# linkedin/ml-ease

Hardware: NVIDIA H100
Metric: ADMM iterations/sec (higher is better)
Workload: dtype f32 data / f64 reductions / bf16 (dense) or e4m3 (CSR) Gram operands

## Files before the change

### ml-ease_b200/csrc/batch.cu

```cuda
#include <algorithm>
#include <cstring>
#include <string>
#include <vector>

#include "host.cuh"

namespace mlease {

namespace {

__global__ void poll2_kernel(const Problem* probs, int nprob, int* flag_out, Problem* compact) {
  __shared__ int s_cnt;
  if (threadIdx.x == 0) s_cnt = 0;
  __syncthreads();
  int running = 0, emit = 0;
  for (int b = threadIdx.x; b < nprob; b += blockDim.x) {
    const Ctrl* c = probs[b].ctrl;
    if (!c->done) {
      running = 1;
      if (c->emit) { emit = 1; compact[atomicAdd(&s_cnt, 1)] = probs[b]; }
    }
  }
  running = __syncthreads_or(running);
  emit = __syncthreads_or(emit);
  if (threadIdx.x == 0) { flag_out[0] = running | (emit << 1); flag_out[1] = s_cnt; }
}

}

static int csr_operand_bytes(int csr_gram) { return csr_gram == CSR_GRAM_SPARSE ? 4 : 1; }
static double gram_path_bytes(const Batch& B) {
  const double Dp = round_up(B.ldx, 128), ldh = round_up(B.Dt, 32);
  double per = Dp * Dp * 4.0 + 3.0 * ldh * ldh * 8.0 + 2.0 * ldh * 32 * 8.0 + (cholesky_factored_direction((int)ldh) ? ldh * ldh * 2.0 : 0.0);
  double bytes = per * B.nprob;
  for (auto& p : B.h) bytes += (double)csr_operand_bytes(B.csr_gram) * (double)p.bm_entries;
  return bytes;
}

constexpr double GRAM_WGMMA_S_PER_MAC = 1.317e-15, GRAM_WGMMA_S_PER_READ = 4.315e-12;
constexpr double GRAM_SPARSE_S_PER_PAIR = 1.808e-12, GRAM_SPARSE_S_PER_VISIT = 2.548e-10, GRAM_SPARSE_S_PER_READ = 2.915e-12;
static double gram_cost(const Problem& p, int Dp, int kind, double ctas, int num_sms) {
  const double nblk = Dp / 128, tiles = nblk * (nblk + 1) / 2, groups = (double)((p.n + 31) / 32);
  const int span = gram_sparse_span(p.bm_entries, Dp / 128, (p.n + 31) / 32);
  const double spans = (double)(((p.n + 31) / 32 + span - 1) / span);
  const double reads = (nblk + 1) * (double)p.bm_entries;
  if (kind == CSR_GRAM_WGMMA) return tiles * 128.0 * 128.0 * 32.0 * groups * GRAM_WGMMA_S_PER_MAC + reads * GRAM_WGMMA_S_PER_READ;
  return (p.gram_pairs * GRAM_SPARSE_S_PER_PAIR + tiles * spans * GRAM_SPARSE_S_PER_VISIT + reads * GRAM_SPARSE_S_PER_READ) *
         std::max(1.0, num_sms / std::max(1.0, ctas));
}

int batch_alloc(Batch& B, int num_sms, int hessian_policy, int csr_gram_force) {
  const int nprob = B.nprob, ldx = B.ldx;
  B.Dp = round_up(B.ldx, 128);
  B.ldh = round_up(B.Dt, 32);
  long long maxn = 1;
  for (auto& p : B.h) maxn = std::max(maxn, p.n);
  int R = 64, cps = 1;
  if (!B.csr) {
    int S, G;
    size_t smem;
    if (!k1_dense_plan(ldx, &R, &S, &G, &smem, &cps))
      return fail(MLEASE_ERR_INVALID, "dense partitions support at most 4095 features (+intercept); use CSR input beyond that");
  }
  const long long row_tiles = (maxn + R - 1) / R;
  B.k1_dyn = (nprob > 1 && nprob <= 32) ? nprob : 0;
  if (B.k1_dyn) B.k1_grid = (int)std::max(1LL, std::min((long long)num_sms * cps, (long long)nprob * row_tiles));
  else B.k1_grid = (int)std::max(1LL, std::min(row_tiles, (long long)std::max(1, (num_sms * cps) / std::max(1, nprob))));
  B.gram_from_csr = B.csr ? 1 : 0;
  for (auto& p : B.h) if (!p.bm_offs) B.gram_from_csr = 0;
  B.csr_fx = B.gram_from_csr;
  if (hessian_policy == 2 && B.csr) {
    B.csr_fx = 1;
    for (auto& p : B.h) if (!p.csr_unique) B.csr_fx = 0;
  }
  B.k1_fused = 0;
  if (B.csr && B.csr_fx && B.group_L >= 1 && B.group_L <= 4 && nprob % B.group_L == 0) {
    bool ok = true;
    for (auto& p : B.h) if (!p.sg_perm || p.sg_S != B.h[0].sg_S || p.sg_rows != B.h[0].sg_rows) ok = false;
    if (ok) {
      B.k1f_LP = B.group_L <= 1 ? 1 : (B.group_L == 2 ? 2 : 4);
      B.k1f_smem = (size_t)ldx * 4 * B.k1f_LP + (size_t)B.h[0].sg_rows * 4 * B.k1f_LP;
      if (B.k1f_smem <= 224 * 1024) { B.k1_fused = 1; B.k1_dyn = 0; B.k1_grid = B.h[0].sg_S; }
    }
  }
  const int gpart_rows = B.k1_fused ? 1 : B.k1_grid;
  if (hessian_policy == 2 && !B.csr)
    return fail(MLEASE_ERR_INVALID, "hessian_policy 2 (matrix-free Newton-CG) needs CSR partitions; dense partitions (at most 4095 features) use the Gram path");
  if (hessian_policy == 2 && !B.csr_fx)
    return fail(MLEASE_ERR_INVALID, "hessian_policy 2 (matrix-free Newton-CG) needs CSR rows with strictly increasing column ids");
  B.matfree = hessian_policy == 2 ? 1 : 0;
  B.csr_gram = 0;
  if (B.gram_from_csr && !B.matfree) {
    double t_sparse = 0, t_wgmma = 0;
    bool fits = true;
    const double nblk = B.Dp / 128, ctas = nblk * (nblk + 1) / 2 * nprob;
    for (auto& p : B.h) {
      t_sparse += gram_cost(p, B.Dp, CSR_GRAM_SPARSE, ctas, num_sms);
      t_wgmma += gram_cost(p, B.Dp, CSR_GRAM_WGMMA, ctas, num_sms);
      if (p.n > gram_sparse_max_rows()) fits = false;
    }
    B.csr_gram = (fits && t_sparse < t_wgmma) ? CSR_GRAM_SPARSE : CSR_GRAM_WGMMA;
    if (csr_gram_force == CSR_GRAM_SPARSE && !fits)
      return fail(MLEASE_ERR_INVALID, "the sparse CSR Gram's int64 sums hold at most 2^27 rows per partition");
    if (csr_gram_force) B.csr_gram = csr_gram_force;
  }
  if (!B.matfree && B.csr && B.gram_from_csr) {
    double state = 0;
    for (auto& p : B.h) state += 8.0 * (double)p.n;
    state += (double)nprob * (8.0 * ((9 + 2 * BFGS_M + gpart_rows) * (double)ldx + B.k1_grid + 8) + 16.0 * ldx +
                              (B.k1_fused ? 4.0 * B.k1_grid * ldx : 0.0));
    size_t free_b = 0, total_b = 0;
    CK(cudaMemGetInfo(&free_b, &total_b));
    if (gram_path_bytes(B) + state + (256.0 * 1024 * 1024) > (double)free_b) { B.matfree = 1; B.csr_gram = 0; }
  }
  {
    double bytes = 0;
    for (auto& p : B.h) bytes = std::max(bytes, B.csr ? 8.0 * (double)p.nnz_hint + 17.0 * (double)p.n : (double)p.n * 4.0 * ldx);
    const double t_pass = bytes / 5e12 + 20e-6;
    const double t_rebuild = (double)maxn * B.Dt * B.Dt / 1e15 + (double)B.Dt * B.Dt * B.Dt / 5e12 + 300e-6;
    B.rebuild_is_expensive = (t_rebuild > 8.0 * t_pass && B.Dt > 2048 && !B.matfree) ? 1 : 0;
  }
  constexpr int MAX_TILES = 1 << 18;
  std::vector<short> tiles(B.matfree ? 2 : 2 * (size_t)MAX_TILES);
  B.ntiles = B.matfree ? 0 : gram_tile_list(B.Dp, tiles.data(), MAX_TILES, B.csr_gram == CSR_GRAM_SPARSE ? 2 : B.gram_from_csr);
  if (B.ntiles <= 0 && !B.matfree) return fail(MLEASE_ERR_INVALID, "Gram tile list overflow");
  if (!B.matfree && B.csr_gram != CSR_GRAM_SPARSE) {
    const long long ksteps = (maxn + 63) / 64;
    const long long base = (long long)B.ntiles * nprob;
    const long long cap = std::max(1, num_sms);
    int best = 1;
    double best_eff = 0;
    for (int s = 1; s <= 16; s++) {
      if (s > ksteps) break;
      const long long ctas = base * s;
      const double eff = (double)ctas / (double)(((ctas + cap - 1) / cap) * cap);
      if (eff > best_eff + 1e-9) { best_eff = eff; best = s; }
      if (eff >= 0.93 && ctas >= 2LL * cap) { best = s; break; }
    }
    while (best > 1 && (double)best * B.Dp * B.Dp * 4.0 * nprob > 1024.0 * 1024 * 1024) best--;
    B.gram_slices = best;
  }
  const size_t nd_prob = ((9 + (B.matfree ? 5 : 2 * BFGS_M)) * (size_t)ldx + 2 * BFGS_M + (size_t)gpart_rows * ldx + (size_t)B.k1_grid + 8 + 3) & ~(size_t)3;
  const size_t nd = (size_t)nprob * nd_prob;
  const size_t nf = (size_t)nprob * 4 * ldx;
  double* dd; float* ff; float* hp = nullptr; double* lc = nullptr; double* ld = nullptr; double* ldi = nullptr; double* yi = nullptr; double* hi = nullptr;
  if (int rc = B.mem.get(&dd, nd, true)) return rc;
  if (int rc = B.mem.get(&ff, nf, true)) return rc;
  float* gpf = nullptr;
  if (B.k1_fused)
    if (int rc = B.mem.get(&gpf, (size_t)nprob * B.k1_grid * ldx, true)) return rc;
  __nv_bfloat16* hif = nullptr;
  if (!B.matfree) {
    if (int rc = B.mem.get(&hp, (size_t)nprob * B.gram_slices * B.Dp * B.Dp, true)) return rc;
    if (int rc = B.mem.get(&lc, (size_t)nprob * B.ldh * B.ldh, true)) return rc;
    if (int rc = B.mem.get(&ld, (size_t)nprob * B.ldh * 32, true)) return rc;
    if (int rc = B.mem.get(&ldi, (size_t)nprob * B.ldh * 32, true)) return rc;
    if (int rc = B.mem.get(&yi, (size_t)nprob * B.ldh * B.ldh, true)) return rc;
    if (int rc = B.mem.get(&hi, (size_t)nprob * B.ldh * B.ldh, true)) return rc;
    if (cholesky_factored_direction(B.ldh))
      if (int rc = B.mem.get(&hif, (size_t)nprob * B.ldh * B.ldh, true)) return rc;
  }
  if (int rc = B.mem.get(&B.d_ctrl, (size_t)nprob, true)) return rc;
  if (int rc = B.mem.get(&B.d, (size_t)nprob, true)) return rc;
  if (nprob > 64 || B.lockstep)
    if (int rc = B.mem.get(&B.d_compact, (size_t)nprob, true)) return rc;
  if (int rc = B.mem.get(&B.d_tmaps, nprob, true)) return rc;
  if (int rc = B.mem.get(&B.d_tiles, (size_t)B.ntiles * 2, true)) return rc;
  CK(cudaMemcpy(B.d_tiles, tiles.data(), (size_t)B.ntiles * 2 * sizeof(short), cudaMemcpyHostToDevice));
  std::vector<CUtensorMap> maps(nprob);
  std::vector<size_t> pool_off(nprob);
  size_t pool_bytes = 0;
  for (int b = 0; b < nprob; b++) {
    pool_off[b] = pool_bytes;
    const bool windows = B.csr_fx && k1_csr_window(ldx) > 0;
    const size_t need = B.csr_fx ? (((size_t)B.h[b].n * sizeof(float) * (windows ? 2 : 1) + 255) & ~(size_t)255) +
                                       (B.matfree ? 0 : (size_t)csr_operand_bytes(B.csr_gram) * (size_t)B.h[b].bm_entries)
                                        : (size_t)B.h[b].n * B.Dp * sizeof(__nv_bfloat16);
    pool_bytes += (need + 255) & ~(size_t)255;
  }
  unsigned char* pool = nullptr;
  if (int rc = B.mem.get(&pool, pool_bytes, true)) return rc;
  for (int b = 0; b < nprob; b++) {
    Problem& p = B.h[b];
    p.ldx = ldx; p.Dt = B.Dt; p.Dp = B.Dp; p.ldh = B.ldh; p.self_idx = b;
    p.k1_ctas = B.k1_grid;
    p.gram_slices = B.gram_slices;
    double* const q0 = dd;
    double* q = dd;
    p.beta = q; q += ldx; p.beta_t = q; q += ldx; p.m = q; q += ldx; p.q = q; q += ldx;
    p.g_t = q; q += ldx; p.g_acc = q; q += ldx; p.dir = q; q += ldx; p.x_d = q; q += ldx;
    p.qf = reinterpret_cast<float*>(q); p.tf = p.qf + ldx; q += ldx;
    if (!B.matfree) { p.bfgs_S = q; q += (size_t)BFGS_M * ldx; p.bfgs_Y = q; q += (size_t)BFGS_M * ldx; }
    p.bfgs_rho = q; q += BFGS_M; p.bfgs_alpha = q; q += BFGS_M;
    p.gpart = q; q += (size_t)gpart_rows * ldx;
    p.hv_vf = p.qf;
    if (B.matfree) { p.cg_r = q; q += ldx; p.cg_p = q; q += ldx; p.cg_z = q; q += ldx; p.cg_Hp = q; q += ldx; p.cg_diag = q; q += ldx; }
    p.gpart_f = gpf ? gpf + (size_t)b * B.k1_grid * ldx : nullptr;
    p.fpart = q; q += B.k1_grid + 8;
    dd = q0 + nd_prob;
    float* f = ff;
    p.beta_tf = f; f += ldx; p.u_f = f; f += ldx; p.uplusx_f = f; f += ldx; p.x_f = f; f += ldx;
    ff = f;
    p.Hpart = hp ? hp + (size_t)b * B.gram_slices * B.Dp * B.Dp : nullptr;
    p.Lc = lc ? lc + (size_t)b * B.ldh * B.ldh : nullptr;
    p.Ldiag = ld ? ld + (size_t)b * B.ldh * 32 : nullptr;
    p.Ldinv = ldi ? ldi + (size_t)b * B.ldh * 32 : nullptr;
    p.Yinv = yi ? yi + (size_t)b * B.ldh * B.ldh : nullptr;
    p.Hinv = hi ? hi + (size_t)b * B.ldh * B.ldh : nullptr;
    p.Ysym = hif ? hif + (size_t)b * B.ldh * B.ldh : nullptr;
    p.ctrl = B.d_ctrl + b;
    if (B.csr_fx) {
      p.sdvec = reinterpret_cast<float*>(pool + pool_off[b]);
      p.rvec = k1_csr_window(ldx) > 0 ? p.sdvec + p.n : nullptr;
      unsigned char* op = B.matfree ? nullptr : pool + pool_off[b] + (((size_t)p.n * sizeof(float) * (p.rvec ? 2 : 1) + 255) & ~(size_t)255);
      p.bm_e4m3 = B.csr_gram == CSR_GRAM_SPARSE ? nullptr : op;
      p.bm_word = B.csr_gram == CSR_GRAM_SPARSE ? reinterpret_cast<uint32_t*>(op) : nullptr;
      p.gram_from_csr = B.gram_from_csr;
      p.csr_gram = B.csr_gram;
      std::memset(&maps[b], 0, sizeof(CUtensorMap));
    } else {
      p.gram_from_csr = 0;
      p.csr_gram = 0;
      p.gram_scale = 1.f; p.gram_unscale = 1.f;
      p.Xt = reinterpret_cast<__nv_bfloat16*>(pool + pool_off[b]);
      if (gram_make_tensor_map(&maps[b], p.Xt, p.n, B.Dp) != 0) return fail(MLEASE_ERR_CUDA, "cuTensorMapEncodeTiled failed");
    }
  }
  CK(cudaMemcpy(B.d_tmaps, maps.data(), (size_t)nprob * sizeof(CUtensorMap), cudaMemcpyHostToDevice));
  CK(cudaMemcpy(B.d, B.h.data(), (size_t)nprob * sizeof(Problem), cudaMemcpyHostToDevice));
  return 0;
}

cudaError_t batch_gram(const Batch& B, const Problem* d_probs, int n, int force, cudaStream_t st, int* launches, int share) {
  if (B.csr_gram == CSR_GRAM_SPARSE) return gram_launch_csr_sparse(d_probs, n, B.d_tiles, B.ntiles, force, st, launches, share);
  if (B.gram_from_csr) return gram_launch_csr_wgmma(d_probs, n, B.d_tiles, B.ntiles, B.gram_slices, force, st, launches, share);
  return gram_launch_wgmma(d_probs, n, B.d_tmaps, B.d_tiles, B.ntiles, B.gram_slices, force, st, launches, share);
}

static double gram_build_flops(const Batch& B, const Problem& p) {
  return B.csr_gram == CSR_GRAM_SPARSE ? 2.0 * p.gram_pairs : (double)p.n * (double)B.Dt * (double)(B.Dt + 1);
}

cudaError_t batch_k1(Batch& B, int force_emit, cudaStream_t st, int* launches, int mode) {
  if (mode != K1_GRAD && !(B.csr && B.csr_fx)) return cudaErrorInvalidValue;
  if (B.k1_fused)
    return k1f_launch(B.d, B.nprob / B.group_L, B.group_L, B.h[0].sg_S, B.k1f_LP, B.k1f_smem, B.has_bias, force_emit, st, launches, mode);
  return k1_launch(B.d, B.nprob, B.csr, B.ldx, B.has_bias, B.k1_grid, force_emit, st, launches, B.csr_fx, B.k1_dyn, mode);
}

int batch_factor(Batch& B, const Problem* d_hess, int n_hess, int share, bool share_fact, int skip_prep, cudaStream_t st, int* launches) {
  if (B.ysym_shared) CK(cholesky_detach_followers(B.d, B.nprob, B.ldh, st, launches));
  if (share_fact) CK(cholesky_share_begin(B.d, B.nprob, share, st, launches));
  CK(cholesky_launch(d_hess, n_hess, B.ldh, st, launches, share, skip_prep));
  if (share_fact) {
    CK(cholesky_share_end(B.d, B.nprob, share, st, launches));
    if (cholesky_factored_direction(B.ldh)) B.ysym_shared = true;
    const size_t hh = (size_t)B.ldh * B.ldh;
    for (int b = 0; b < B.nprob; b++) {
      if (b % share == 0) continue;
      const Problem& lead = B.h[b - b % share];
      if (!cholesky_factored_direction(B.ldh)) CK(cudaMemcpyAsync(B.h[b].Hinv, lead.Hinv, hh * sizeof(double), cudaMemcpyDeviceToDevice, st));
    }
  }
  B.has_factor = true;
  return 0;
}

static int mf_direction(Batch& B, const SlotCtx& x) {
  constexpr int CG_CHUNK = 4;
  Profiler& pf = *x.pf;
  cudaStream_t st = x.st;
  int& launches = *x.launches;
  pf.begin(2, st);
  CK(cg_begin(B.d, B.nprob, st, &launches));
  CK(batch_k1(B, 0, st, &launches, K1_DIAG));
  CK(hv_reduce(B.d, B.nprob, B.Dt, 2, st, &launches));
  CK(cg_init(B.d, B.nprob, B.Dt, st, &launches));
  pf.end(st);
  for (int steps = 0; steps < CG_MAX_STEPS; steps += CG_CHUNK) {
    for (int j = 0; j < CG_CHUNK; j++) {
      pf.begin(2, st);
      CK(batch_k1(B, 0, st, &launches, K1_HV));
      CK(hv_reduce(B.d, B.nprob, B.Dt, 1, st, &launches));
      CK(cg_step(B.d, B.nprob, B.Dt, st, &launches));
      pf.end(st);
    }
    CK(cg_poll(B.d, B.nprob, x.d_flag + 2, st, &launches));
    CK(cudaMemcpyAsync(x.h_flag + 2, x.d_flag + 2, sizeof(int), cudaMemcpyDeviceToHost, st));
    CK(cudaStreamSynchronize(st));
    if (!x.h_flag[2]) break;
  }
  return 0;
}

int batch_slot(Batch& B, const SlotCtx& x, int slot_idx, bool with_hess, bool spec) {
  Profiler& pf = *x.pf;
  cudaStream_t st = x.st;
  int& launches = *x.launches;
  pf.begin(0, st);
  CK(batch_k1(B, B.matfree ? 1 : -1, st, &launches));
  pf.end(st);
  pf.begin(1, st);
  CK(k1_reduce_decide(B.d, B.nprob, B.Dt, st, &launches, spec ? 1 : 0));
  pf.end(st);
  if (with_hess && x.n_hess > 0) {
    pf.begin(2, st);
    const int share = (slot_idx == 0) ? x.share_first_gram : 0;
    if (share > 1)
      for (int b = 0; b < B.nprob; b++) if (b % share != 0) *x.shared_flops += gram_build_flops(B, B.h[b]);
    CK(batch_gram(B, x.d_hess, x.n_hess, 0, st, &launches, share));
    pf.end(st);
    pf.begin(3, st);
    const bool share_fact = share > 1 && x.share_first_factor;
    if (int rc = batch_factor(B, x.d_hess, x.n_hess, share, share_fact, 0, st, &launches)) return rc;
    pf.end(st);
  }
  if (B.matfree)
    if (int rc = mf_direction(B, x)) return rc;
  pf.begin(1, st);
  if (B.matfree) CK(newton_finish(B.d, B.nprob, B.Dt, st, &launches));
  else CK(newton_solve(B.d, B.nprob, B.ldh, st, &launches, B.group_L));
  if (x.poll) { poll2_kernel<<<1, 256, 0, st>>>(B.d, B.nprob, x.d_flag, B.d_compact); launches++; }
  pf.end(st);
  return 0;
}

int batch_xupdate(Batch& B, cudaStream_t st, double xtol, int max_newton, int policy, int invalidate, int* h_flag, int* d_flag,
                  Counters& cnt, Profiler* prof, int share_first_gram, int share_first_factor) {
  Profiler nop;
  Profiler& pf = prof ? *prof : nop;
  int launches = 0;
  if (B.matfree) policy = 2;
  CK(newton_begin(B.d, B.nprob, xtol, max_newton, policy, invalidate, B.rebuild_is_expensive, st, &launches));
  const bool small = B.nprob <= 64 && !B.lockstep;
  int flag = 1;
  {
    bool emit0 = policy == 1 || invalidate || B.mirror.empty();
    for (auto& c : B.mirror) if (!c.hess_valid || c.refresh_next) emit0 = true;
    if (emit0 && !B.matfree) flag |= 2;
  }
  B.mirror.resize(B.nprob);
  std::vector<Ctrl>& hc = B.mirror;
  int slots = 0;
  const Problem* d_hess = B.d;
  int n_hess = B.nprob;
  double shared_flops = 0;
  auto enqueue_slot = [&](int slot_idx, bool with_hess, bool spec) -> int {
    const SlotCtx x{st, &pf, &launches, d_hess, n_hess, share_first_gram, share_first_factor, &shared_flops, h_flag, d_flag, !small};
    return batch_slot(B, x, slot_idx, with_hess, spec);
  };
  if (small) {
    for (int i = 0; i < 2; i++) {
      if (!B.h_ctrl[i]) if (int rc = B.pinned.get(&B.h_ctrl[i], B.nprob, false)) return rc;
      if (!B.slot_ev[i]) CK(cudaEventCreateWithFlags(&B.slot_ev[i], cudaEventDisableTiming));
    }
    const bool may_spec = policy == 0;
    auto flags_of = [&](const Ctrl* c, bool* all_valid) {
      int f = 0; bool v = true;
      for (int b = 0; b < B.nprob; b++) if (!c[b].done) { f |= 1; if (c[b].emit) f |= 2; if (!c[b].hess_valid) v = false; }
      *all_valid = v;
      return f;
    };
    auto finish_slot = [&](int idx) -> int {
      CK(cudaMemcpyAsync(B.h_ctrl[idx & 1], B.d_ctrl, (size_t)B.nprob * sizeof(Ctrl), cudaMemcpyDeviceToHost, st));
      CK(cudaEventRecord(B.slot_ev[idx & 1], st));
      return 0;
    };
    bool known_valid = !(flag & 2);
    if (int rc = enqueue_slot(0, (flag & 2) != 0, false)) return rc;
    if (int rc = finish_slot(0)) return rc;
    int s_cur = 0;
    bool next_in_flight = false;
    int known_flag = flag;
    while (true) {
      const bool spec_next = may_spec && known_valid && !(known_flag & 2) && s_cur + 1 < 400;
      if (spec_next) {
        if (int rc = enqueue_slot(s_cur + 1, false, true)) return rc;
        if (int rc = finish_slot(s_cur + 1)) return rc;
        next_in_flight = true;
      }
      CK(cudaEventSynchronize(B.slot_ev[s_cur & 1]));
      std::memcpy(hc.data(), B.h_ctrl[s_cur & 1], (size_t)B.nprob * sizeof(Ctrl));
      slots = s_cur + 1;
      known_flag = flags_of(hc.data(), &known_valid);
      if (!(known_flag & 1) || slots >= 400) break;
      if (next_in_flight) { s_cur++; next_in_flight = false; continue; }
      if (int rc = enqueue_slot(s_cur + 1, (known_flag & 2) != 0, false)) return rc;
      if (int rc = finish_slot(s_cur + 1)) return rc;
      s_cur++;
    }
    flag = known_flag;
  }
  while (!small && (flag & 1) && slots < 400) {
    if (int rc = enqueue_slot(slots, (flag & 2) != 0, false)) return rc;
    CK(cudaMemcpyAsync(h_flag, d_flag, 2 * sizeof(int), cudaMemcpyDeviceToHost, st));
    CK(cudaStreamSynchronize(st));
    flag = h_flag[0];
    n_hess = h_flag[1];
    d_hess = B.d_compact;
    slots++;
  }
  if (!small) {
    CK(cudaMemcpyAsync(hc.data(), B.d_ctrl, (size_t)B.nprob * sizeof(Ctrl), cudaMemcpyDeviceToHost, st));
    CK(cudaStreamSynchronize(st));
  }
  cnt.launches += launches;
  cnt.last_slots = slots;
  int bad_spd = 0, bad_ls = 0;
  if (pf.on) CK(cudaStreamSynchronize(st));
  pf.resolve();
  for (int b = 0; b < B.nprob; b++) {
    const Ctrl& c = hc[b];
    const Problem& p = B.h[b];
    const double rowbytes = B.csr ? 17.0 : (4.0 * B.ldx + 9.0);
    cnt.k1_bytes += (double)c.evals * ((double)p.n * rowbytes + (B.csr ? 8.0 * (double)p.nnz_hint : 0.0));
    cnt.gram_flops += (double)c.hess_builds * gram_build_flops(B, p);
    cnt.k1_emit_bytes += (double)c.hess_builds * (double)p.n * (double)B.Dp * 2.0;
  }
  cnt.gram_flops -= shared_flops;
  if (B.csr) {
    const int gl = std::max(1, B.group_L);
    for (int g0 = 0; g0 + gl <= B.nprob; g0 += gl) {
      int mx = 0; long long sum = 0;
      for (int l = 0; l < gl; l++) { mx = std::max(mx, hc[g0 + l].evals); sum += hc[g0 + l].evals; }
      const Problem& p = B.h[g0];
      cnt.k1_shared_bytes += (double)mx * (8.0 * (double)p.nnz_hint + 9.0 * (double)p.n) + (double)sum * 8.0 * (double)p.n;
    }
  }
  for (auto& c : hc) {
    cnt.k1_passes += c.evals; cnt.newton_steps += c.newton_steps; cnt.rejected += c.rejects; cnt.gram_builds += c.hess_builds;
    if (c.fail == 3 || !c.done) cnt.not_converged++;
    if (c.fail == 1) bad_spd++;
    if (c.fail == 2) bad_ls++;
  }
  if (bad_spd) return fail(MLEASE_ERR_NUMERIC, "Model fitting error! (Hessian not positive definite in " + std::to_string(bad_spd) + " problem(s))");
  if (bad_ls) return fail(MLEASE_ERR_NUMERIC, "Model fitting error! (line search failed in " + std::to_string(bad_ls) + " problem(s))");
  return 0;
}

}
```

### ml-ease_b200/csrc/common.cuh

```cuda
#pragma once
#include <cuda_bf16.h>
#include <cuda_runtime.h>
#include <stdint.h>

namespace mlease {

constexpr int BFGS_M = 6;
constexpr int CG_MAX_STEPS = 64;

struct Ctrl {
  int done;
  int have_dir;
  int need_solve;
  int need_hess;
  int emit;
  int hess_valid;
  int fail;
  int newton_steps;
  int evals;
  int rejects;
  int hess_builds;
  int stall;
  int bfgs_count;
  double h0_scale;
  int k1_chunks;
  int refresh_next;
  int skip_eval;
  int warm_used;
  int build_step;
  double worst_ratio;
  double alpha;
  double phi0;
  double f_acc, f_t;
  double gnorm;
  double gnorm_prev;
  double dirnorm;
  double dirnorm_prev;
  double xtol;
  int max_newton;
  int hess_policy;
  int rebuild_is_expensive;
  long long tot_evals, tot_newton, tot_rejects, tot_hess;
  const void* ysym_use;
  int cg_active;
  int cg_iter;
  double cg_rz;
  double cg_g2;
  float hv_vinf;
};

enum { K1_GRAD = 0, K1_HV = 1, K1_DIAG = 2 };
enum { CSR_GRAM_WGMMA = 1, CSR_GRAM_SPARSE = 2 };

struct Problem {
  const float* X;
  long long n;
  int ldx;
  int Dt;
  const signed char* y;
  const float* w;
  const float* o;
  const long long* rowptr;
  const int* colidx;
  const float* vals;
  long long nnz_hint;
  int csr_unique;
  const long long* bm_offs;
  const unsigned short* bm_keys;
  const float* bm_vals;
  long long bm_groups;
  long long bm_entries;
  unsigned char* bm_e4m3;
  uint32_t* bm_word;
  float vmax, wmax;
  int nblk128;
  int sg_S, sg_rows, sg_ngrp;
  const int* sg_perm;
  const int* sg_depth;
  const long long* sg_goff;
  const unsigned short* sg_row16;
  const float* sg_val;
  const unsigned short* sg_col16;
  float* gpart_f;
  float* sdvec;
  float* rvec;
  int gram_from_csr;
  int csr_gram;
  double gram_pairs;
  float gram_scale;
  float gram_unscale;
  __nv_bfloat16* Xt;
  int Dp;
  double* beta;
  double* beta_t;
  float* beta_tf;
  double* m;
  double* q;
  double* g_t;
  double* g_acc;
  double* dir;
  double* gpart;
  double* fpart;
  int k1_ctas;
  float* Hpart;
  int gram_slices;
  double* Lc;
  double* Ldiag;
  double* Ldinv;
  double* Yinv;
  double* Hinv;
  __nv_bfloat16* Ysym;
  float* qf;
  float* tf;
  int ldh;
  Ctrl* ctrl;
  float* u_f;
  float* uplusx_f;
  float* x_f;
  double* bfgs_S;
  double* bfgs_Y;
  double* bfgs_rho;
  double* bfgs_alpha;
  double* x_d;
  int lambda_idx;
  int self_idx;
  int part_local;
  float rowl1;
  float* hv_vf;
  double* cg_r;
  double* cg_p;
  double* cg_z;
  double* cg_Hp;
  double* cg_diag;
};

__device__ __forceinline__ uint32_t smem_u32(const void* p) { return (uint32_t)__cvta_generic_to_shared(p); }

__device__ __forceinline__ void mbar_init(uint64_t* bar, uint32_t count) {
  asm volatile("mbarrier.init.shared::cta.b64 [%0], %1;" ::"r"(smem_u32(bar)), "r"(count) : "memory");
}
__device__ __forceinline__ void fence_mbar_init() { asm volatile("fence.mbarrier_init.release.cluster;" ::: "memory"); }
__device__ __forceinline__ void fence_proxy_async_smem() { asm volatile("fence.proxy.async.shared::cta;" ::: "memory"); }
__device__ __forceinline__ void mbar_arrive_expect_tx(uint64_t* bar, uint32_t bytes) {
  asm volatile("mbarrier.arrive.expect_tx.shared::cta.b64 _, [%0], %1;" ::"r"(smem_u32(bar)), "r"(bytes) : "memory");
}
__device__ __forceinline__ void mbar_arrive(uint64_t* bar) {
  asm volatile("mbarrier.arrive.shared::cta.b64 _, [%0];" ::"r"(smem_u32(bar)) : "memory");
}
__device__ __forceinline__ bool mbar_try_wait(uint64_t* bar, uint32_t parity) {
  uint32_t ok;
  asm volatile(
      "{\n"
      ".reg .pred p;\n"
      "mbarrier.try_wait.parity.shared::cta.b64 p, [%1], %2;\n"
      "selp.u32 %0, 1, 0, p;\n"
      "}\n"
      : "=r"(ok)
      : "r"(smem_u32(bar)), "r"(parity)
      : "memory");
  return ok != 0;
}
__device__ __forceinline__ void mbar_wait(uint64_t* bar, uint32_t parity) {
  while (!mbar_try_wait(bar, parity)) {
  }
}
__device__ __forceinline__ void mbar_arrive(uint32_t bar) { asm volatile("mbarrier.arrive.shared::cta.b64 _, [%0];" ::"r"(bar) : "memory"); }
__device__ __forceinline__ void mbar_wait(uint32_t bar, uint32_t parity) {
  uint32_t ok;
  do {
    asm volatile(
        "{\n"
        ".reg .pred p;\n"
        "mbarrier.try_wait.parity.shared::cta.b64 p, [%1], %2;\n"
        "selp.u32 %0, 1, 0, p;\n"
        "}\n"
        : "=r"(ok)
        : "r"(bar), "r"(parity)
        : "memory");
  } while (!ok);
}

__device__ __forceinline__ void sts_u8(uint32_t saddr, uint32_t v) { asm volatile("st.shared.u8 [%0], %1;" ::"r"(saddr), "r"(v) : "memory"); }
__device__ __forceinline__ void bulk_g2s(void* dst_smem, const void* src_gmem, uint32_t bytes, uint64_t* bar) {
  asm volatile("cp.async.bulk.shared::cluster.global.mbarrier::complete_tx::bytes [%0], [%1], %2, [%3];" ::"r"(
                   smem_u32(dst_smem)),
               "l"(src_gmem), "r"(bytes), "r"(smem_u32(bar))
               : "memory");
}

__device__ __forceinline__ void tma_load_2d(void* dst_smem, const void* tmap, int c0, int c1, uint64_t* bar) {
  asm volatile(
      "cp.async.bulk.tensor.2d.shared::cluster.global.tile.mbarrier::complete_tx::bytes [%0], [%1, {%2, %3}], [%4];" ::"r"(
          smem_u32(dst_smem)),
      "l"(tmap), "r"(c0), "r"(c1), "r"(smem_u32(bar))
      : "memory");
}
__device__ __forceinline__ void tma_prefetch_desc(const void* tmap) {
  asm volatile("prefetch.tensormap [%0];" ::"l"(tmap) : "memory");
}

__device__ __forceinline__ uint64_t wgmma_desc(uint32_t smem_addr, uint32_t lbo_bytes, uint32_t sbo_bytes, uint32_t layout) {
  uint64_t d = 0;
  d |= (uint64_t)((smem_addr & 0x3FFFF) >> 4);
  d |= (uint64_t)((lbo_bytes >> 4) & 0x3FFF) << 16;
  d |= (uint64_t)((sbo_bytes >> 4) & 0x3FFF) << 32;
  d |= (uint64_t)(layout & 3) << 62;
  return d;
}
__device__ __forceinline__ void wgmma_fence() { asm volatile("wgmma.fence.sync.aligned;" ::: "memory"); }
__device__ __forceinline__ void wgmma_commit() { asm volatile("wgmma.commit_group.sync.aligned;" ::: "memory"); }
template <int N>
__device__ __forceinline__ void wgmma_wait() { asm volatile("wgmma.wait_group.sync.aligned %0;" ::"n"(N) : "memory"); }
__device__ __forceinline__ void wgmma_bf16_m64n256k16_tt(float (&d)[128], uint64_t desc_a, uint64_t desc_b) {
  asm volatile(
      "{\n"
      ".reg .pred p;\n"
      "setp.ne.b32 p, 1, 0;\n"
      "wgmma.mma_async.sync.aligned.m64n256k16.f32.bf16.bf16 {"
      "%0, %1, %2, %3, %4, %5, %6, %7, %8, %9, %10, %11, %12, %13, %14, %15, "
      "%16, %17, %18, %19, %20, %21, %22, %23, %24, %25, %26, %27, %28, %29, %30, %31, "
      "%32, %33, %34, %35, %36, %37, %38, %39, %40, %41, %42, %43, %44, %45, %46, %47, "
      "%48, %49, %50, %51, %52, %53, %54, %55, %56, %57, %58, %59, %60, %61, %62, %63, "
      "%64, %65, %66, %67, %68, %69, %70, %71, %72, %73, %74, %75, %76, %77, %78, %79, "
      "%80, %81, %82, %83, %84, %85, %86, %87, %88, %89, %90, %91, %92, %93, %94, %95, "
      "%96, %97, %98, %99, %100, %101, %102, %103, %104, %105, %106, %107, %108, %109, %110, %111, "
      "%112, %113, %114, %115, %116, %117, %118, %119, %120, %121, %122, %123, %124, %125, %126, %127}, "
      "%128, %129, p, 1, 1, 1, 1;\n"
      "}\n"
      : "+f"(d[0]), "+f"(d[1]), "+f"(d[2]), "+f"(d[3]), "+f"(d[4]), "+f"(d[5]), "+f"(d[6]), "+f"(d[7]),
        "+f"(d[8]), "+f"(d[9]), "+f"(d[10]), "+f"(d[11]), "+f"(d[12]), "+f"(d[13]), "+f"(d[14]), "+f"(d[15]),
        "+f"(d[16]), "+f"(d[17]), "+f"(d[18]), "+f"(d[19]), "+f"(d[20]), "+f"(d[21]), "+f"(d[22]), "+f"(d[23]),
        "+f"(d[24]), "+f"(d[25]), "+f"(d[26]), "+f"(d[27]), "+f"(d[28]), "+f"(d[29]), "+f"(d[30]), "+f"(d[31]),
        "+f"(d[32]), "+f"(d[33]), "+f"(d[34]), "+f"(d[35]), "+f"(d[36]), "+f"(d[37]), "+f"(d[38]), "+f"(d[39]),
        "+f"(d[40]), "+f"(d[41]), "+f"(d[42]), "+f"(d[43]), "+f"(d[44]), "+f"(d[45]), "+f"(d[46]), "+f"(d[47]),
        "+f"(d[48]), "+f"(d[49]), "+f"(d[50]), "+f"(d[51]), "+f"(d[52]), "+f"(d[53]), "+f"(d[54]), "+f"(d[55]),
        "+f"(d[56]), "+f"(d[57]), "+f"(d[58]), "+f"(d[59]), "+f"(d[60]), "+f"(d[61]), "+f"(d[62]), "+f"(d[63]),
        "+f"(d[64]), "+f"(d[65]), "+f"(d[66]), "+f"(d[67]), "+f"(d[68]), "+f"(d[69]), "+f"(d[70]), "+f"(d[71]),
        "+f"(d[72]), "+f"(d[73]), "+f"(d[74]), "+f"(d[75]), "+f"(d[76]), "+f"(d[77]), "+f"(d[78]), "+f"(d[79]),
        "+f"(d[80]), "+f"(d[81]), "+f"(d[82]), "+f"(d[83]), "+f"(d[84]), "+f"(d[85]), "+f"(d[86]), "+f"(d[87]),
        "+f"(d[88]), "+f"(d[89]), "+f"(d[90]), "+f"(d[91]), "+f"(d[92]), "+f"(d[93]), "+f"(d[94]), "+f"(d[95]),
        "+f"(d[96]), "+f"(d[97]), "+f"(d[98]), "+f"(d[99]), "+f"(d[100]), "+f"(d[101]), "+f"(d[102]), "+f"(d[103]),
        "+f"(d[104]), "+f"(d[105]), "+f"(d[106]), "+f"(d[107]), "+f"(d[108]), "+f"(d[109]), "+f"(d[110]), "+f"(d[111]),
        "+f"(d[112]), "+f"(d[113]), "+f"(d[114]), "+f"(d[115]), "+f"(d[116]), "+f"(d[117]), "+f"(d[118]), "+f"(d[119]),
        "+f"(d[120]), "+f"(d[121]), "+f"(d[122]), "+f"(d[123]), "+f"(d[124]), "+f"(d[125]), "+f"(d[126]), "+f"(d[127])
      : "l"(desc_a), "l"(desc_b)
      : "memory");
}
__device__ __forceinline__ void wgmma_e4m3_m64n128k32(float (&d)[64], uint64_t desc_a, uint64_t desc_b, uint32_t accumulate) {
  asm volatile(
      "{\n"
      ".reg .pred p;\n"
      "setp.ne.b32 p, %66, 0;\n"
      "wgmma.mma_async.sync.aligned.m64n128k32.f32.e4m3.e4m3 {"
      "%0, %1, %2, %3, %4, %5, %6, %7, %8, %9, %10, %11, %12, %13, %14, %15, "
      "%16, %17, %18, %19, %20, %21, %22, %23, %24, %25, %26, %27, %28, %29, %30, %31, "
      "%32, %33, %34, %35, %36, %37, %38, %39, %40, %41, %42, %43, %44, %45, %46, %47, "
      "%48, %49, %50, %51, %52, %53, %54, %55, %56, %57, %58, %59, %60, %61, %62, %63}, "
      "%64, %65, p, 1, 1;\n"
      "}\n"
      : "+f"(d[0]), "+f"(d[1]), "+f"(d[2]), "+f"(d[3]), "+f"(d[4]), "+f"(d[5]), "+f"(d[6]), "+f"(d[7]),
        "+f"(d[8]), "+f"(d[9]), "+f"(d[10]), "+f"(d[11]), "+f"(d[12]), "+f"(d[13]), "+f"(d[14]), "+f"(d[15]),
        "+f"(d[16]), "+f"(d[17]), "+f"(d[18]), "+f"(d[19]), "+f"(d[20]), "+f"(d[21]), "+f"(d[22]), "+f"(d[23]),
        "+f"(d[24]), "+f"(d[25]), "+f"(d[26]), "+f"(d[27]), "+f"(d[28]), "+f"(d[29]), "+f"(d[30]), "+f"(d[31]),
        "+f"(d[32]), "+f"(d[33]), "+f"(d[34]), "+f"(d[35]), "+f"(d[36]), "+f"(d[37]), "+f"(d[38]), "+f"(d[39]),
        "+f"(d[40]), "+f"(d[41]), "+f"(d[42]), "+f"(d[43]), "+f"(d[44]), "+f"(d[45]), "+f"(d[46]), "+f"(d[47]),
        "+f"(d[48]), "+f"(d[49]), "+f"(d[50]), "+f"(d[51]), "+f"(d[52]), "+f"(d[53]), "+f"(d[54]), "+f"(d[55]),
        "+f"(d[56]), "+f"(d[57]), "+f"(d[58]), "+f"(d[59]), "+f"(d[60]), "+f"(d[61]), "+f"(d[62]), "+f"(d[63])
      : "l"(desc_a), "l"(desc_b), "r"(accumulate)
      : "memory");
}

template <int N>
__device__ __forceinline__ void setmaxnreg_dec() { asm volatile("setmaxnreg.dec.sync.aligned.u32 %0;" ::"n"(N)); }
template <int N>
__device__ __forceinline__ void setmaxnreg_inc() { asm volatile("setmaxnreg.inc.sync.aligned.u32 %0;" ::"n"(N)); }

__device__ __forceinline__ float warp_sum(float v) {
#pragma unroll
  for (int o = 16; o > 0; o >>= 1) v += __shfl_xor_sync(0xffffffffu, v, o);
  return v;
}
__device__ __forceinline__ double warp_sum(double v) {
#pragma unroll
  for (int o = 16; o > 0; o >>= 1) v += __shfl_xor_sync(0xffffffffu, v, o);
  return v;
}
__device__ __forceinline__ double warp_max(double v) {
#pragma unroll
  for (int o = 16; o > 0; o >>= 1) v = fmax(v, __shfl_xor_sync(0xffffffffu, v, o));
  return v;
}

}
```

### ml-ease_b200/csrc/ingest.cu

```cuda
#include <algorithm>
#include <cstring>
#include <string>

#include "host.cuh"

namespace mlease {

namespace {

__global__ void fill_bias_pad_kernel(float* X, long long n, int ldx, int Dg, int has_bias) {
  const int npad = ldx - Dg;
  const long long total = n * npad;
  for (long long e = (long long)blockIdx.x * blockDim.x + threadIdx.x; e < total; e += (long long)gridDim.x * blockDim.x) {
    const long long i = e / npad;
    const int c = Dg + (int)(e % npad);
    X[i * ldx + c] = (c == Dg && has_bias) ? 1.0f : 0.0f;
  }
}
__global__ void convert_labels_kernel(long long n, const int* resp, const float* w_in, const float* o_in, signed char* y, float* w,
                                      float* o, int* bad) {
  for (long long i = (long long)blockIdx.x * blockDim.x + threadIdx.x; i < n; i += (long long)gridDim.x * blockDim.x) {
    const int r = resp[i];
    if (r != 1 && r != 0 && r != -1) atomicOr(bad, 1);
    y[i] = (r == 1) ? 1 : -1;
    const float ww = w_in ? w_in[i] : 1.0f;
    if (!(ww >= 0.f)) atomicOr(bad, 2);
    w[i] = ww;
    o[i] = o_in ? o_in[i] : 0.0f;
  }
}
__global__ void check_rows_sorted_kernel(long long n, const long long* rowptr, const int* colidx, int* bad) {
  for (long long i = (long long)blockIdx.x * blockDim.x + threadIdx.x; i < n; i += (long long)gridDim.x * blockDim.x)
    for (long long j = rowptr[i] + 1; j < rowptr[i + 1]; j++)
      if (colidx[j] <= colidx[j - 1]) { atomicOr(bad, 8); break; }
}
__global__ void absmax_kernel(long long n, const float* __restrict__ a, unsigned* __restrict__ out) {
  float m = 0.f;
  for (long long j = (long long)blockIdx.x * blockDim.x + threadIdx.x; j < n; j += (long long)gridDim.x * blockDim.x) m = fmaxf(m, fabsf(a[j]));
  m = warp_max(m);
  if ((threadIdx.x & 31) == 0) atomicMax(out, __float_as_uint(m));
}
__global__ void csr_gram_pairs_kernel(long long n, const long long* __restrict__ rowptr, unsigned long long* __restrict__ out) {
  unsigned long long s = 0;
  for (long long i = (long long)blockIdx.x * blockDim.x + threadIdx.x; i < n; i += (long long)gridDim.x * blockDim.x) {
    const unsigned long long k = (unsigned long long)(rowptr[i + 1] - rowptr[i]);
    s += (k + 1) * (k + 2) / 2;
  }
  for (int d = 16; d > 0; d >>= 1) s += __shfl_down_sync(0xffffffffu, s, d);
  if ((threadIdx.x & 31) == 0) atomicAdd(out, s);
}
__global__ void check_csr_kernel(long long nnz, const int* colidx, float* vals, int Dg, int binary, int* bad) {
  for (long long j = (long long)blockIdx.x * blockDim.x + threadIdx.x; j < nnz; j += (long long)gridDim.x * blockDim.x) {
    const int c = colidx[j];
    if (c < 0 || c >= Dg) atomicOr(bad, 4);
    if (binary) vals[j] = 1.0f;
  }
}
__global__ void gather_i64_kernel(const long long* src, const long long* idx, int n, long long* out) {
  const int i = blockIdx.x * blockDim.x + threadIdx.x;
  if (i < n) out[i] = src[idx[i]];
}
__global__ void rebase_rowptr_kernel(long long n, const long long* src, long long base, long long* dst) {
  for (long long i = (long long)blockIdx.x * blockDim.x + threadIdx.x; i <= n; i += (long long)gridDim.x * blockDim.x) dst[i] = src[i] - base;
}
__global__ void repack_rows_kernel(float* dst, int ldx, const float* src, long long ld_in, long long rows, int Dg) {
  const long long total = rows * Dg;
  for (long long e = (long long)blockIdx.x * blockDim.x + threadIdx.x; e < total; e += (long long)gridDim.x * blockDim.x) {
    const long long i = e / Dg;
    const int c = (int)(e - i * Dg);
    dst[i * ldx + c] = src[i * ld_in + c];
  }
}

}

bool is_device_ptr(const void* p) {
  cudaPointerAttributes a;
  const bool dev = cudaPointerGetAttributes(&a, p) == cudaSuccess && (a.type == cudaMemoryTypeDevice || a.type == cudaMemoryTypeManaged);
  cudaGetLastError();
  return dev;
}

bool is_dma_ptr(const void* p) {
  cudaPointerAttributes a;
  const bool dma = cudaPointerGetAttributes(&a, p) == cudaSuccess &&
                   (a.type == cudaMemoryTypeDevice || a.type == cudaMemoryTypeManaged || a.type == cudaMemoryTypeHost);
  cudaGetLastError();
  return dma;
}

int gather_rowptr(const int64_t* rowptr, const std::vector<long long>& idx, std::vector<long long>& out) {
  out.resize(idx.size());
  if (!is_device_ptr(rowptr)) {
    for (size_t i = 0; i < idx.size(); i++) out[i] = rowptr[idx[i]];
    return 0;
  }
  DevMem t;
  long long *d_idx, *d_out;
  if (int rc = t.get(&d_idx, idx.size(), false)) return rc;
  if (int rc = t.get(&d_out, idx.size(), false)) return rc;
  CK(cudaMemcpy(d_idx, idx.data(), idx.size() * 8, cudaMemcpyHostToDevice));
  gather_i64_kernel<<<(int)((idx.size() + 255) / 256), 256>>>((const long long*)rowptr, d_idx, (int)idx.size(), d_out);
  CK(cudaMemcpy(out.data(), d_out, idx.size() * 8, cudaMemcpyDeviceToHost));
  return 0;
}

int ingest_labels(cudaStream_t st, long long n, const int32_t* response, const float* weight, const float* offset, signed char* y, float* w,
                  float* o, int* d_flag, int* h_flag, float* wmax) {
  DevMem t;
  const int* d_r; const float *d_w, *d_o;
  if (int rc = to_device(t, (const int*)response, (size_t)n, &d_r, st)) return rc;
  if (int rc = to_device(t, weight, (size_t)n, &d_w, st)) return rc;
  if (int rc = to_device(t, offset, (size_t)n, &d_o, st)) return rc;
  CK(cudaMemsetAsync(d_flag, 0, 8, st));
  if (n > 0) {
    convert_labels_kernel<<<(int)std::min<long long>((n + 255) / 256, 4096), 256, 0, st>>>(n, d_r, d_w, d_o, y, w, o, d_flag);
    if (wmax) absmax_kernel<<<(int)std::min<long long>((n + 255) / 256, 2048), 256, 0, st>>>(n, w, (unsigned*)(d_flag + 1));
  }
  CK(cudaMemcpyAsync(h_flag, d_flag, 8, cudaMemcpyDeviceToHost, st));
  CK(cudaStreamSynchronize(st));
  if (h_flag[0] & 1) return fail(MLEASE_ERR_INVALID, "response (only 1, 0, -1 are allowed)");
  if (h_flag[0] & 2) return fail(MLEASE_ERR_INVALID, "weight cannot < 0");
  if (wmax && n > 0) std::memcpy(wmax, h_flag + 1, 4);
  return 0;
}

void check_csr(cudaStream_t st, long long n, long long nnz, const long long* rowptr, const int* colidx, float* vals, int Dg, int binary,
               int* d_flag) {
  if (nnz <= 0) return;
  check_csr_kernel<<<(int)std::min<long long>((nnz + 255) / 256, 4096), 256, 0, st>>>(nnz, colidx, vals, Dg, binary, d_flag);
  check_rows_sorted_kernel<<<(int)std::min<long long>((n + 255) / 256, 4096), 256, 0, st>>>(n, rowptr, colidx, d_flag + 1);
}

void rebase_rowptr(cudaStream_t st, long long n, const long long* src, long long base, long long* dst) {
  rebase_rowptr_kernel<<<(int)std::min<long long>((n + 256) / 256, 4096), 256, 0, st>>>(n, src, base, dst);
}

int upload_dense_rows(float* dst, int ldx, const float* src, long long ld_in, long long n, int Dg, int has_bias, cudaStream_t st) {
  if (is_device_ptr(src)) {
    repack_rows_kernel<<<4096, 256, 0, st>>>(dst, ldx, src, ld_in, n, Dg);
  } else {
    const long long chunk_rows = std::max<long long>(1, (128LL << 20) / (ld_in * 4));
    struct Staging {
      cudaEvent_t h2d_done[2] = {nullptr, nullptr}, repack_done[2] = {nullptr, nullptr};
      cudaStream_t cs = nullptr;
      ~Staging() {
        for (int b = 0; b < 2; b++) { if (h2d_done[b]) cudaEventDestroy(h2d_done[b]); if (repack_done[b]) cudaEventDestroy(repack_done[b]); }
        if (cs) cudaStreamDestroy(cs);
      }
    } sg;
    DevMem bufs;
    float* buf[2];
    CK(cudaStreamCreateWithFlags(&sg.cs, cudaStreamNonBlocking));
    for (int b = 0; b < 2; b++) {
      if (int rc = bufs.get(&buf[b], (size_t)chunk_rows * ld_in, false)) return rc;
      CK(cudaEventCreateWithFlags(&sg.h2d_done[b], cudaEventDisableTiming));
      CK(cudaEventCreateWithFlags(&sg.repack_done[b], cudaEventDisableTiming));
    }
    int ci = 0;
    for (long long r0 = 0; r0 < n; r0 += chunk_rows, ci++) {
      const int b = ci & 1;
      const long long rows = std::min(chunk_rows, n - r0);
      if (ci >= 2) CK(cudaStreamWaitEvent(sg.cs, sg.repack_done[b], 0));
      const size_t bytes = ((size_t)(rows - 1) * ld_in + Dg) * 4;
      CK(cudaMemcpyAsync(buf[b], src + r0 * ld_in, bytes, cudaMemcpyHostToDevice, sg.cs));
      CK(cudaEventRecord(sg.h2d_done[b], sg.cs));
      CK(cudaStreamWaitEvent(st, sg.h2d_done[b], 0));
      repack_rows_kernel<<<2048, 256, 0, st>>>(dst + r0 * ldx, ldx, buf[b], ld_in, rows, Dg);
      CK(cudaEventRecord(sg.repack_done[b], st));
    }
    CK(cudaStreamSynchronize(sg.cs));
    CK(cudaStreamSynchronize(st));
  }
  fill_bias_pad_kernel<<<1024, 256, 0, st>>>(dst, n, ldx, Dg, has_bias);
  return 0;
}

int csr_build_layout(mlease_session* s, PartData& pd) {
  Problem& d = pd.data;
  if (d.nnz_hint <= 0) return 0;
  const long long nrows = d.n, nnz = d.nnz_hint;
  const std::string who = "partition " + std::to_string(pd.pid) + ": ";
  int* f = s->d_flag;
  CK(cudaMemsetAsync(f, 0, 24, s->stream));
  check_csr(s->stream, nrows, nnz, d.rowptr, d.colidx, const_cast<float*>(d.vals), s->Dg, s->cfg.binary_feature, f);
  absmax_kernel<<<(int)std::min<long long>((nnz + 255) / 256, 2048), 256, 0, s->stream>>>(nnz, d.vals, (unsigned*)(f + 2));
  CK(csr_row_l1_max(nrows, d.rowptr, d.vals, (unsigned*)(f + 3), s->stream));
  csr_gram_pairs_kernel<<<(int)std::min<long long>((nrows + 255) / 256, 2048), 256, 0, s->stream>>>(nrows, d.rowptr, (unsigned long long*)(f + 4));
  CK(cudaMemcpyAsync(s->h_flag, f, 24, cudaMemcpyDeviceToHost, s->stream));
  CK(cudaStreamSynchronize(s->stream));
  if (s->h_flag[0]) return fail(MLEASE_ERR_INVALID, who + "feature index out of range");
  d.csr_unique = s->h_flag[1] ? 0 : 1;
  std::memcpy(&d.vmax, s->h_flag + 2, 4);
  std::memcpy(&d.rowl1, s->h_flag + 3, 4);
  unsigned long long pairs = 0;
  std::memcpy(&pairs, s->h_flag + 4, 8);
  if (d.csr_unique && nnz + nrows < (1LL << 32) - 64 && s->cfg.hessian_policy != 2) {
    d.nblk128 = round_up(s->ldx, 128) / 128;
    d.bm_groups = (nrows + 31) / 32;
    d.bm_entries = nnz + nrows;
    long long* bo; unsigned short* bk; float* bv;
    if (int rc = s->mem.get(&bo, (size_t)d.nblk128 * d.bm_groups + 1, true)) return rc;
    if (int rc = s->mem.get(&bk, (size_t)d.bm_entries, true)) return rc;
    if (int rc = s->mem.get(&bv, (size_t)d.bm_entries, true)) return rc;
    CK(csr_bm_offsets(nrows, d.rowptr, d.colidx, s->Dg, d.nblk128, d.bm_groups, bo, s->stream));
    CK(csr_bm_fill(nrows, d.rowptr, d.colidx, d.vals, s->Dg, d.nblk128, d.bm_groups, bo, bk, bv, s->stream));
    d.bm_offs = bo; d.bm_keys = bk; d.bm_vals = bv;
    d.gram_pairs = (double)pairs;
  }
  if (d.csr_unique && nnz + nrows < (1LL << 32) - 64) {
    int S = 0, rows = 0, LP = 0; size_t smem = 0;
    if (k1f_plan(nrows, s->ldx, s->L, s->num_sms, &S, &rows, &LP, &smem)) {
      int *perm, *depth; long long* goff; unsigned short *row16, *col16; float* val; long long total;
      CK(k1f_build(nrows, s->Dg, nnz, d.rowptr, d.colidx, d.vals, S, rows, &d.sg_ngrp, &perm, &depth, &goff, &row16, &val, &total, &col16,
                   s->stream));
      d.sg_S = S; d.sg_rows = rows;
      d.sg_perm = perm; d.sg_depth = depth; d.sg_goff = goff; d.sg_row16 = row16; d.sg_val = val; d.sg_col16 = col16;
      for (void* p : {(void*)perm, (void*)depth, (void*)goff, (void*)row16, (void*)val, (void*)col16}) s->mem.adopt(p);
    }
  }
  return 0;
}

}
```

### ml-ease_b200/csrc/k2_gram.cu

```cuda
#include <cuda.h>
#include <cuda_fp8.h>

#include <algorithm>
#include <cub/device/device_scan.cuh>

#include "kernels.cuh"

namespace mlease {

constexpr int GM = 128;
constexpr int GN = 256;
constexpr int GK = 64;
constexpr int UK = 16;
constexpr int GSTAGES = 4;
constexpr int G_A_BYTES = GK * GM * 2;
constexpr int G_B_BYTES = GK * GN * 2;
constexpr int G_STAGE_BYTES = G_A_BYTES + G_B_BYTES;
constexpr int G_BOX_BYTES = GK * 64 * 2;
constexpr int G_THREADS = 384;
constexpr size_t G_SMEM = (size_t)GSTAGES * G_STAGE_BYTES + 1024  + 256 ;
constexpr uint32_t DESC_SW128 = 1, DESC_SW32 = 3;

struct GramTile { short bi, bj; };

template <int N>
__device__ __forceinline__ void store_acc(float* out, int Dp, int row0, int col0, const float (&d)[N / 2]) {
  const int lane = threadIdx.x & 31, w = (threadIdx.x >> 5) & 3;
  const int r = row0 + w * 16 + (lane >> 2);
  if (r + 8 >= Dp) return;
#pragma unroll
  for (int j = 0; j < N / 8; j++) {
    const int c = col0 + 8 * j + 2 * (lane & 3);
    if (c < Dp) {
      *reinterpret_cast<float2*>(out + (size_t)r * Dp + c) = make_float2(d[4 * j], d[4 * j + 1]);
      *reinterpret_cast<float2*>(out + (size_t)(r + 8) * Dp + c) = make_float2(d[4 * j + 2], d[4 * j + 3]);
    }
  }
}

__global__ void __launch_bounds__(G_THREADS, 1)
gram_wgmma_kernel(const Problem* __restrict__ probs, const CUtensorMap* __restrict__ tmaps, const GramTile* __restrict__ tiles,
                  int ntiles, int force, int share) {
  if (share > 1 && blockIdx.z % share != 0) return;
  const int pidx = blockIdx.z;
  const Problem& pb = probs[pidx];
  Ctrl* ctrl = pb.ctrl;
  if (!force && (ctrl->done || !ctrl->need_hess)) return;
  const CUtensorMap* tmap = &tmaps[pb.self_idx];
  const GramTile tile = tiles[blockIdx.x];
  const int slice = blockIdx.y, nslices = gridDim.y;
  const int Dp = pb.Dp;
  const long long ksteps_total = (pb.n + GK - 1) / GK;
  const long long per = (ksteps_total + nslices - 1) / nslices;
  const long long ks0 = slice * per;
  const long long ks1 = min(ksteps_total, ks0 + per);
  const int nk = (int)max(0LL, ks1 - ks0);

  extern __shared__ unsigned char g_smem_raw[];
  unsigned char* smem = reinterpret_cast<unsigned char*>((reinterpret_cast<uintptr_t>(g_smem_raw) + 1023) & ~uintptr_t(1023));
  uint64_t* full_bar = reinterpret_cast<uint64_t*>(smem + (size_t)GSTAGES * G_STAGE_BYTES);
  uint64_t* empty_bar = full_bar + GSTAGES;

  const int lane = threadIdx.x & 31, wg = threadIdx.x >> 7;

  if (threadIdx.x == 0) {
    tma_prefetch_desc(tmap);
    for (int s = 0; s < GSTAGES; s++) { mbar_init(&full_bar[s], 1); mbar_init(&empty_bar[s], 8); }
    fence_mbar_init();
  }
  __syncthreads();

  if (wg == 0) {
    if (threadIdx.x == 0) {
      for (int k = 0; k < nk; k++) {
        const int st = k % GSTAGES;
        if (k >= GSTAGES) mbar_wait(&empty_bar[st], (uint32_t)(((k / GSTAGES) - 1) & 1));
        unsigned char* a_dst = smem + (size_t)st * G_STAGE_BYTES;
        unsigned char* b_dst = a_dst + G_A_BYTES;
        mbar_arrive_expect_tx(&full_bar[st], G_STAGE_BYTES);
        const int krow = (int)((ks0 + k) * GK);
#pragma unroll
        for (int b = 0; b < GM / 64; b++) tma_load_2d(a_dst + b * G_BOX_BYTES, tmap, tile.bi * GM + b * 64, krow, &full_bar[st]);
#pragma unroll
        for (int b = 0; b < GN / 64; b++) tma_load_2d(b_dst + b * G_BOX_BYTES, tmap, tile.bj * GN + b * 64, krow, &full_bar[st]);
      }
    }
  } else {
    float acc[GN / 2];
#pragma unroll
    for (int j = 0; j < GN / 2; j++) acc[j] = 0.f;
    const uint32_t smem_base = smem_u32(smem);
    for (int k = 0; k < nk; k++) {
      const int st = k % GSTAGES;
      mbar_wait(&full_bar[st], (uint32_t)((k / GSTAGES) & 1));
      const uint32_t a_addr = smem_base + (uint32_t)(st * G_STAGE_BYTES + (wg - 1) * G_BOX_BYTES);
      const uint32_t b_addr = smem_base + (uint32_t)(st * G_STAGE_BYTES + G_A_BYTES);
      wgmma_fence();
#pragma unroll
      for (int kk = 0; kk < GK / UK; kk++)
        wgmma_bf16_m64n256k16_tt(acc, wgmma_desc(a_addr + kk * (UK * 128), G_BOX_BYTES, 1024, DESC_SW128),
                                 wgmma_desc(b_addr + kk * (UK * 128), G_BOX_BYTES, 1024, DESC_SW128));
      wgmma_commit();
      wgmma_wait<1>();
      if (k > 0 && lane == 0) mbar_arrive(&empty_bar[(k - 1) % GSTAGES]);
    }
    wgmma_wait<0>();
    store_acc<GN>(pb.Hpart + (size_t)slice * Dp * Dp, Dp, tile.bi * GM + (wg - 1) * 64, tile.bj * GN, acc);
  }
}

constexpr int SK = 32;
constexpr int SN = 128;
constexpr int S_BOX_BYTES = SK * 128;
constexpr int SPW = 2;
constexpr int NGRP = 4;
constexpr int SST = 2 * NGRP;
constexpr int S_STAGE_BYTES = SPW * S_BOX_BYTES;
constexpr int S_CONSUMER_WARPS = 8;
constexpr int S_THREADS = (S_CONSUMER_WARPS + SPW * NGRP) * 32;
constexpr int S_CHAIN = 4;
static_assert(SST == 2 * S_CHAIN, "the consumer loop runs two chains per pass over the ring");
constexpr int S_REG_PRODUCER = 72, S_REG_CONSUMER = 184;
constexpr size_t S_SMEM = (size_t)SST * S_STAGE_BYTES + 1024  + 512 ;

__device__ __forceinline__ uint32_t kmaj_off(int k, int col) {
  return (uint32_t)(col * 32 + ((((k >> 4) ^ (col >> 2)) & 1) << 4) + (k & 15));
}
__device__ __forceinline__ int kmaj_row(uint32_t key) { return (int)(((((key >> 4) ^ (key >> 7)) & 1) << 4) | (key & 15)); }

__global__ void __launch_bounds__(S_THREADS, 1)
gram_csr_wgmma_kernel(const Problem* __restrict__ probs, const GramTile* __restrict__ tiles, int ntiles, int force, int share) {
  if (share > 1 && blockIdx.z % share != 0) return;
  const Problem& pb = probs[blockIdx.z];
  Ctrl* ctrl = pb.ctrl;
  if (!force && (ctrl->done || !ctrl->need_hess)) return;
  const GramTile tile = tiles[blockIdx.x];
  const int slice = blockIdx.y, nslices = gridDim.y;
  const int Dp = pb.Dp;
  const long long ksteps_total = (pb.n + SK - 1) / SK;
  const long long per = (ksteps_total + nslices - 1) / nslices;
  const long long ks0 = slice * per;
  const long long ks1 = min(ksteps_total, ks0 + per);
  const int nk = (int)max(0LL, ks1 - ks0);

  extern __shared__ unsigned char g_smem_raw[];
  unsigned char* smem = reinterpret_cast<unsigned char*>((reinterpret_cast<uintptr_t>(g_smem_raw) + 1023) & ~uintptr_t(1023));
  uint64_t* full_bar = reinterpret_cast<uint64_t*>(smem + (size_t)SST * S_STAGE_BYTES);
  uint64_t* empty_bar = full_bar + SST;
  const uint32_t smem_base = smem_u32(smem);
  const uint32_t full_u32 = smem_base + (uint32_t)SST * S_STAGE_BYTES, empty_u32 = full_u32 + 8 * SST;
  const int warp = threadIdx.x >> 5, lane = threadIdx.x & 31;

  for (int e = threadIdx.x; e < SST * S_STAGE_BYTES / 16; e += S_THREADS) reinterpret_cast<uint4*>(smem)[e] = make_uint4(0u, 0u, 0u, 0u);
  if (threadIdx.x == 0) {
    for (int s = 0; s < SST; s++) { mbar_init(&full_bar[s], SPW); mbar_init(&empty_bar[s], S_CONSUMER_WARPS); }
    fence_mbar_init();
  }
  fence_proxy_async_smem();
  __syncthreads();

  if (warp < S_CONSUMER_WARPS) {
    setmaxnreg_inc<S_REG_CONSUMER>();
    const int wg = warp >> 2;
    float acc[SN / 2], chain[SN / 2];
#pragma unroll
    for (int j = 0; j < SN / 2; j++) acc[j] = 0.f;
    const uint64_t desc_a0 = wgmma_desc(smem_base + (uint32_t)(wg * 64 * SK), 16, 256, DESC_SW32);
    const uint64_t desc_b0 = wgmma_desc(smem_base + (uint32_t)S_BOX_BYTES, 16, 256, DESC_SW32);
    const uint32_t desc_hi = (uint32_t)(desc_a0 >> 32);
    uint32_t a_lo = (uint32_t)desc_a0, b_lo = (uint32_t)desc_b0;
    asm volatile("" : "+r"(a_lo), "+r"(b_lo));
    auto desc_a = [&](int st) { return ((uint64_t)desc_hi << 32) | (a_lo + (uint32_t)(st * S_STAGE_BYTES / 16)); };
    auto desc_b = [&](int st) { return ((uint64_t)desc_hi << 32) | (b_lo + (uint32_t)(st * S_STAGE_BYTES / 16)); };
    auto issue = [&](int st, uint32_t ph, uint64_t a, uint64_t b, uint32_t accumulate) {
      mbar_wait(full_u32 + 8 * st, ph);
      wgmma_fence();
      wgmma_e4m3_m64n128k32(chain, a, b, accumulate);
      wgmma_commit();
    };
    auto release = [&](int st) { if (lane == 0) mbar_arrive(empty_u32 + 8 * st); };
    auto promote = [&]() {
#pragma unroll
      for (int j = 0; j < SN / 2; j++) acc[j] += chain[j];
    };
    auto run_chain = [&](int s0, uint32_t ph) {
#pragma unroll
      for (int c = 0; c < S_CHAIN; c++) {
        issue(s0 + c, ph, desc_a(s0 + c), desc_b(s0 + c), c != 0 ? 1u : 0u);
        if (c > 0) { wgmma_wait<1>(); release(s0 + c - 1); }
      }
      wgmma_wait<0>();
      release(s0 + S_CHAIN - 1);
      promote();
    };
    const int nring = nk - nk % SST, nfull = nk - nk % S_CHAIN;
    uint32_t ph = 0;
    int k = 0;
    for (; k < nring; k += SST) {
      run_chain(0, ph);
      run_chain(S_CHAIN, ph);
      ph ^= 1u;
    }
    if (k < nfull) { run_chain(0, ph); k += S_CHAIN; }
    for (; k < nk; k++) {
      const int st = k % SST;
      issue(st, (uint32_t)(k / SST) & 1u, desc_a(st), desc_b(st), 0u);
      wgmma_wait<0>();
      release(st);
      promote();
    }
    store_acc<SN>(pb.Hpart + (size_t)slice * Dp * Dp, Dp, tile.bi * 128 + wg * 64, tile.bj * SN, acc);
  } else {
    setmaxnreg_dec<S_REG_PRODUCER>();
    const int pw = warp - S_CONSUMER_WARPS;
    const int grp = pw / SPW, strm = pw % SPW;
    const int blk = strm == 0 ? tile.bi : tile.bj;
    const bool valid = blk < pb.nblk128;
    const long long* __restrict__ my_offs = pb.bm_offs + (size_t)(valid ? blk : 0) * pb.bm_groups + ks0 + (lane & 1);
    const unsigned short* __restrict__ keys = pb.bm_keys;
    const unsigned char* __restrict__ bytes = pb.bm_e4m3;
    constexpr uint32_t NOKEY = 0xFFFFFFFFu;
    const bool fetch = valid && lane < 2;
    auto ld_offs = [&](int k) -> uint32_t { return (fetch && k < nk) ? (uint32_t)__ldg(my_offs + k) : 0u; };

    struct Run { uint32_t lo, hi, key[2], byte[2]; };
    struct Written { uint32_t lo, hi, key[2]; };
    auto take_offs = [&](Run& r, uint32_t o) { r.lo = __shfl_sync(0xffffffffu, o, 0); r.hi = __shfl_sync(0xffffffffu, o, 1); };
    auto ld_entries = [&](Run& r) {
#pragma unroll
      for (int q = 0; q < 2; q++) {
        const uint32_t e = r.lo + lane + 32 * q;
        r.key[q] = e < r.hi ? (uint32_t)__ldg(keys + e) : NOKEY;
        r.byte[q] = e < r.hi ? (uint32_t)__ldg(bytes + e) : 0u;
      }
    };
    Run r0, r1;
    Written w0 = {0u, 0u, {NOKEY, NOKEY}}, w1 = {0u, 0u, {NOKEY, NOKEY}};
    take_offs(r0, ld_offs(grp));
    take_offs(r1, ld_offs(grp + NGRP));
    uint32_t o_c = ld_offs(grp + 2 * NGRP);
    ld_entries(r0);
    ld_entries(r1);
    const uint32_t sbase0 = smem_base + (uint32_t)(grp * S_STAGE_BYTES + strm * S_BOX_BYTES), sbase1 = sbase0 + NGRP * S_STAGE_BYTES;
    const uint32_t full0 = full_u32 + 8 * grp, empty0 = empty_u32 + 8 * grp;
    auto use = [&](int k, uint32_t sbase, uint32_t full, uint32_t empty, bool refill, uint32_t ph, Run& r, Written& w) {
      if (refill) {
        mbar_wait(empty, ph);
#pragma unroll
        for (int q = 0; q < 2; q++)
          if (w.key[q] != NOKEY) sts_u8(sbase + w.key[q], 0u);
        for (uint32_t e0 = w.lo + 64; e0 < w.hi; e0 += 32) {
          const uint32_t e = e0 + lane;
          if (e < w.hi) sts_u8(sbase + (uint32_t)__ldg(keys + e), 0u);
        }
      }
#pragma unroll
      for (int q = 0; q < 2; q++)
        if (r.key[q] != NOKEY) sts_u8(sbase + r.key[q], r.byte[q]);
      for (uint32_t e0 = r.lo + 64; e0 < r.hi; e0 += 32) {
        const uint32_t e = e0 + lane;
        if (e < r.hi) sts_u8(sbase + (uint32_t)__ldg(keys + e), (uint32_t)__ldg(bytes + e));
      }
      fence_proxy_async_smem();
      __syncwarp();
      if (lane == 0) mbar_arrive(full);
      w.lo = r.lo; w.hi = r.hi; w.key[0] = r.key[0]; w.key[1] = r.key[1];
      take_offs(r, o_c);
      o_c = ld_offs(k + 3 * NGRP);
      ld_entries(r);
    };
    uint32_t ph = 1u;
    for (int k = grp; k < nk; k += SST) {
      use(k, sbase0, full0, empty0, k >= SST, ph, r0, w0);
      if (k + NGRP >= nk) break;
      use(k + NGRP, sbase1, full0 + 8 * NGRP, empty0 + 8 * NGRP, k >= SST, ph, r1, w1);
      ph ^= 1u;
    }
  }
}

__device__ __forceinline__ int e4m3_units(uint32_t b) {
  const int e = (int)((b >> 3) & 15u), m = (int)(b & 7u);
  const int mag = e ? (8 | m) << (e - 1) : m;
  return (b & 0x80u) ? -mag : mag;
}

constexpr uint32_t SW_VALUE_MASK = 0xFFFF8000u;
__device__ __forceinline__ uint32_t sparse_word(uint32_t byte, int row_in_span, int col) {
  return __float_as_uint((float)e4m3_units(byte)) | ((uint32_t)row_in_span << 7) | (uint32_t)col;
}
__device__ __forceinline__ int sw_units(uint32_t w) { return __float2int_rz(__uint_as_float(w & SW_VALUE_MASK)); }
__device__ __forceinline__ int sw_row(uint32_t w) { return (int)((w >> 7) & 255u); }
__device__ __forceinline__ int sw_col(uint32_t w) { return (int)(w & 127u); }

__global__ void __launch_bounds__(256) gram_csr_operand_kernel(const Problem* __restrict__ probs, int force, int share) {
  if (share > 1 && blockIdx.y % share != 0) return;
  const Problem& pb = probs[blockIdx.y];
  const Ctrl* ctrl = pb.ctrl;
  if (!force && (ctrl->done || !ctrl->need_hess)) return;
  const int lane = threadIdx.x & 31;
  const long long n = pb.n, ngroups = pb.bm_groups;
  const int nblk = pb.nblk128;
  const long long* __restrict__ offs = pb.bm_offs;
  const unsigned short* __restrict__ keys = pb.bm_keys;
  const float* __restrict__ vals = pb.bm_vals;
  unsigned char* __restrict__ out = pb.bm_e4m3;
  uint32_t* __restrict__ out_w = pb.bm_word;
  const bool word = pb.csr_gram == CSR_GRAM_SPARSE;
  const int span = gram_sparse_span(pb.bm_entries, nblk, ngroups);
  const float gscale = pb.gram_scale;
  const long long nw = ((long long)gridDim.x * blockDim.x) >> 5;
  for (long long g = ((long long)blockIdx.x * blockDim.x + threadIdx.x) >> 5; g < ngroups; g += nw) {
    const long long r = g * SK + lane;
    const float sd = r < n ? pb.sdvec[r] * gscale : 0.f;
    const int row0 = 32 * (int)(g % span);
    for (int b = 0; b < nblk; b++) {
      const uint32_t lo = (uint32_t)offs[(size_t)b * ngroups + g], hi = (uint32_t)offs[(size_t)b * ngroups + g + 1];
      for (uint32_t e0 = lo; e0 < hi; e0 += 32) {
        const uint32_t e = e0 + lane;
        const bool v = e < hi;
        const uint32_t key = v ? (uint32_t)keys[e] : 0u;
        const float val = v ? vals[e] : 0.f;
        const int k = kmaj_row(key);
        const float sdk = __shfl_sync(0xffffffffu, sd, k);
        const uint32_t byte = __nv_cvt_float_to_fp8(val * sdk, __NV_SATFINITE, __NV_E4M3);
        if (!v) continue;
        if (word) out_w[e] = sparse_word(byte, row0 + k, (int)(key >> 5));
        else out[e] = (unsigned char)byte;
      }
    }
  }
}

constexpr int SP_THREADS = 1024;
constexpr int SP_WARPS = SP_THREADS / 32;
constexpr int SP_SPAN = 8;
constexpr int SP_ROWS = SP_SPAN * 32;
constexpr int SP_AHEAD = 1;
constexpr int SP_STAGE = 448;
constexpr size_t SP_ACC_BYTES = (size_t)SN * SN * 2 * sizeof(uint32_t);
constexpr size_t SP_WARP_BYTES = (size_t)SP_STAGE * 4 + (size_t)SP_ROWS * 4 + 32 * 8;
constexpr size_t SP_SMEM = SP_ACC_BYTES + (size_t)SP_WARPS * SP_WARP_BYTES;
static_assert(SP_SMEM <= 227 * 1024, "sparse Gram shared memory");
static_assert(SP_STAGE % 16 == 0, "layout of the stage");
static_assert(SP_SPAN == 8 && SP_STAGE == 448, "gram_sparse_span (kernels.cuh) assumes these");
static_assert(SP_ROWS <= 256, "sparse_word holds the row in the span in 8 bits");

__global__ void __launch_bounds__(SP_THREADS, 1)
gram_csr_sparse_kernel(const Problem* __restrict__ probs, const GramTile* __restrict__ tiles, int force, int share) {
  if (share > 1 && blockIdx.z % share != 0) return;
  const Problem& pb = probs[blockIdx.z];
  Ctrl* ctrl = pb.ctrl;
  if (!force && (ctrl->done || !ctrl->need_hess)) return;
  const GramTile tile = tiles[blockIdx.x];
  const int bi = tile.bi, bj = tile.bj;
  const bool diag = bi == bj;
  const int Dp = pb.Dp;
  const long long ngroups = pb.bm_groups;
  const int span = gram_sparse_span(pb.bm_entries, pb.nblk128, ngroups);
  const long long nspans = (ngroups + span - 1) / span;
  const int hot = diag && (pb.Dt - 1) / SN == bi ? (pb.Dt - 1) % SN : -1;

  extern __shared__ __align__(16) unsigned char g_smem_raw[];
  uint32_t* acc_lo = reinterpret_cast<uint32_t*>(g_smem_raw);
  int* acc_hi = reinterpret_cast<int*>(g_smem_raw) + SN * SN;
  const int warp = threadIdx.x >> 5, lane = threadIdx.x & 31;
  unsigned char* wsm = g_smem_raw + SP_ACC_BYTES + (size_t)warp * SP_WARP_BYTES;
  int* stage = reinterpret_cast<int*>(wsm);
  uint32_t* rtab = reinterpret_cast<uint32_t*>(wsm + SP_STAGE * 4);
  unsigned short* rtab16 = reinterpret_cast<unsigned short*>(rtab);
  int2* own = reinterpret_cast<int2*>(wsm + SP_STAGE * 4 + SP_ROWS * 4);

  for (int e = threadIdx.x; e < SN * SN; e += SP_THREADS) { acc_lo[e] = 0u; acc_hi[e] = 0; }
  __syncthreads();

  const bool valid = bi < pb.nblk128 && bj < pb.nblk128;
  const long long* __restrict__ offs_i = pb.bm_offs + (size_t)bi * ngroups;
  const long long* __restrict__ offs_j = pb.bm_offs + (size_t)bj * ngroups;
  const uint32_t* __restrict__ words = pb.bm_word;
  const uint32_t lt = (1u << lane) - 1u;
  auto add_cell = [&](int cell, long long p) {
    const uint32_t lo = (uint32_t)p;
    const uint32_t old = atomicAdd(acc_lo + cell, lo);
    const int hi = (int)(p >> 32) + (old + lo < old ? 1 : 0);
    if (hi != 0) atomicAdd(acc_hi + cell, hi);
  };
  auto ld_bounds = [&](long long s) -> uint32_t {
    if (!valid || s >= nspans || lane >= 4) return 0u;
    return (uint32_t)__ldg((lane < 2 ? offs_i : offs_j) + min(s * span + (lane & 1) * span, ngroups));
  };
  auto ld_entry = [&](uint32_t e, uint32_t hi) -> uint32_t { return e < hi ? __ldg(words + e) : 0u; };
  struct Span { uint32_t ilo, ihi, jlo, jhi, i[SP_AHEAD], j[SP_AHEAD]; };
  auto take = [&](Span& q, uint32_t b) {
    q.ilo = __shfl_sync(0xffffffffu, b, 0); q.ihi = __shfl_sync(0xffffffffu, b, 1);
    q.jlo = __shfl_sync(0xffffffffu, b, 2); q.jhi = __shfl_sync(0xffffffffu, b, 3);
#pragma unroll
    for (int k = 0; k < SP_AHEAD; k++) { q.i[k] = ld_entry(q.ilo + lane + 32 * k, q.ihi); q.j[k] = ld_entry(q.jlo + lane + 32 * k, q.jhi); }
  };
  long long hot_sum = 0;
  auto run = [&](const Span& q) {
    const uint32_t ilo = q.ilo, ihi = q.ihi, jlo = q.jlo, jhi = q.jhi;
    if (ilo == ihi || jlo == jhi) return;
    for (uint32_t c0 = jlo; c0 < jhi; c0 += SP_STAGE) {
      const uint32_t c1 = min(jhi, c0 + SP_STAGE);
      __syncwarp();
#pragma unroll
      for (int k = 0; k < SP_ROWS / 128; k++) reinterpret_cast<uint4*>(rtab)[lane + 32 * k] = make_uint4(0u, 0u, 0u, 0u);
      __syncwarp();
      int nst = 0, prev_row = -1;
      uint32_t x[SP_AHEAD + 1];
#pragma unroll
      for (int k = 0; k < SP_AHEAD; k++) x[k] = c0 == jlo ? q.j[k] : ld_entry(c0 + 32 * k + lane, c1);
      for (uint32_t base = c0; base < c1; base += 32) {
        x[SP_AHEAD] = ld_entry(base + 32 * SP_AHEAD + lane, c1);
        const uint32_t w = x[0];
        const int v = sw_units(w);
        const int r = sw_row(w);
        const bool keep = v != 0;
        const uint32_t m = __ballot_sync(0xffffffffu, keep);
        const uint32_t below = m & lt;
        const int up = __shfl_sync(0xffffffffu, r, below ? 31 - __clz(below) : 0);
        const int pr = below ? up : prev_row;
        const int s = nst + __popc(below);
        if (keep) {
          stage[s] = v * 128 + sw_col(w);
          if (r != pr) { rtab16[2 * r] = (unsigned short)s; if (pr >= 0) rtab16[2 * pr + 1] = (unsigned short)s; }
        }
        if (m) prev_row = __shfl_sync(0xffffffffu, r, 31 - __clz(m));
        nst += __popc(m);
#pragma unroll
        for (int k = 0; k < SP_AHEAD; k++) x[k] = x[k + 1];
      }
      if (nst == 0) continue;
      if (lane == 0) rtab16[2 * prev_row + 1] = (unsigned short)nst;
      __syncwarp();
#pragma unroll
      for (int k = 0; k < SP_AHEAD; k++) x[k] = q.i[k];
      for (uint32_t base = ilo; base < ihi; base += 32) {
        x[SP_AHEAD] = ld_entry(base + 32 * SP_AHEAD + lane, ihi);
        const uint32_t w = x[0];
        const int a = sw_units(w);
        const uint32_t t = a != 0 ? rtab[sw_row(w)] : 0u;
        const int s0 = (int)(t & 0xFFFFu), cnt = (int)(t >> 16) - s0;
        int incl = cnt;
#pragma unroll
        for (int d = 1; d < 32; d <<= 1) {
          const int u = __shfl_up_sync(0xffffffffu, incl, d);
          if (lane >= d) incl += u;
        }
        const int total = __shfl_sync(0xffffffffu, incl, 31);
#pragma unroll
        for (int k = 0; k < SP_AHEAD; k++) x[k] = x[k + 1];
        if (total == 0) continue;
        const uint32_t owners = __ballot_sync(0xffffffffu, cnt > 0);
        __syncwarp();
        if (cnt > 0) own[__popc(owners & lt)] = make_int2(a * 128 + sw_col(w), s0 - (incl - cnt));
        __syncwarp();
        int before = 0;
        for (int p0 = 0; p0 < total; p0 += 32) {
          const int end = incl - p0;
          const uint32_t ends = __reduce_or_sync(0xffffffffu, cnt > 0 && end >= 0 && end < 32 ? 1u << end : 0u);
          const int p = p0 + lane;
          if (p < total) {
            const int2 o = own[before + __popc(ends & (0xFFFFFFFFu >> (31 - lane)))];
            const int pv = stage[p + o.y];
            const int c1 = o.x & 127, c2 = pv & 127;
            if (!diag || c2 <= c1) {
              const long long prod = (long long)(o.x >> 7) * (long long)(pv >> 7);
              if (c2 == hot && c1 == hot) hot_sum += prod;
              else add_cell(c1 * SN + c2, prod);
            }
          }
          before += __popc(ends);
        }
      }
    }
  };
  Span cur, nxt;
  take(cur, ld_bounds(warp));
  uint32_t nb = ld_bounds(warp + SP_WARPS);
  for (long long s = warp; s < nspans; s += SP_WARPS) {
    take(nxt, nb);
    nb = ld_bounds(s + 2 * SP_WARPS);
    run(cur);
    cur = nxt;
  }
  if (hot >= 0) {
#pragma unroll
    for (int d = 16; d > 0; d >>= 1) hot_sum += __shfl_down_sync(0xffffffffu, hot_sum, d);
    if (lane == 0 && hot_sum != 0) add_cell(hot * SN + hot, hot_sum);
  }
  __syncthreads();
  float* out = pb.Hpart + (size_t)bi * SN * Dp + (size_t)bj * SN;
  for (int e = threadIdx.x; e < SN * SN; e += SP_THREADS) {
    const int c1 = e >> 7, c2 = e & 127;
    const int idx = diag && c2 > c1 ? c2 * SN + c1 : e;
    const long long v = (long long)(((unsigned long long)(uint32_t)acc_hi[idx] << 32) | acc_lo[idx]);
    out[(size_t)c1 * Dp + c2] = __ll2float_rn(v) * 0x1p-18f;
  }
}

long long gram_sparse_max_rows() { return 1LL << 27; }

__device__ __forceinline__ bool bias_in_block(long long r, long long n, int bias_col, int b) {
  return r < n && bias_col >= b * 128 && bias_col < b * 128 + 128;
}

__global__ void __launch_bounds__(256) csr_bm_count_kernel(long long n, const long long* __restrict__ rowptr, const int* __restrict__ colidx,
                                                           int bias_col, int nblk, long long ngroups, long long* __restrict__ counts) {
  const int lane = threadIdx.x & 31;
  const long long nw = ((long long)gridDim.x * blockDim.x) >> 5;
  for (long long g = ((long long)blockIdx.x * blockDim.x + threadIdx.x) >> 5; g < ngroups; g += nw) {
    const long long r = g * 32 + lane;
    long long j = r < n ? rowptr[r] : 0;
    const long long j1 = r < n ? rowptr[r + 1] : 0;
    for (int b = 0; b < nblk; b++) {
      const long long s = j;
      while (j < j1 && colidx[j] < (b + 1) * 128) j++;
      int c = (int)(j - s) + (bias_in_block(r, n, bias_col, b) ? 1 : 0);
      c = __reduce_add_sync(0xffffffffu, c);
      if (lane == 0) counts[(size_t)b * ngroups + g] = c;
    }
  }
}

__global__ void __launch_bounds__(256) csr_bm_fill_kernel(long long n, const long long* __restrict__ rowptr, const int* __restrict__ colidx,
                                                          const float* __restrict__ vals, int bias_col, int nblk, long long ngroups,
                                                          const long long* __restrict__ offs, unsigned short* __restrict__ keys,
                                                          float* __restrict__ bvals) {
  const int lane = threadIdx.x & 31;
  const long long nw = ((long long)gridDim.x * blockDim.x) >> 5;
  for (long long g = ((long long)blockIdx.x * blockDim.x + threadIdx.x) >> 5; g < ngroups; g += nw) {
    const long long r = g * 32 + lane;
    long long j = r < n ? rowptr[r] : 0;
    const long long j1 = r < n ? rowptr[r + 1] : 0;
    for (int b = 0; b < nblk; b++) {
      const long long s = j;
      while (j < j1 && colidx[j] < (b + 1) * 128) j++;
      const bool bias = bias_in_block(r, n, bias_col, b);
      const int c = (int)(j - s) + (bias ? 1 : 0);
      int incl = c;
#pragma unroll
      for (int d = 1; d < 32; d <<= 1) {
        const int t = __shfl_up_sync(0xffffffffu, incl, d);
        if (lane >= d) incl += t;
      }
      long long pos = offs[(size_t)b * ngroups + g] + (incl - c);
      for (long long e = s; e < j; e++, pos++) {
        keys[pos] = (unsigned short)kmaj_off(lane, colidx[e] - b * 128);
        bvals[pos] = vals[e];
      }
      if (bias) {
        keys[pos] = (unsigned short)kmaj_off(lane, bias_col - b * 128);
        bvals[pos] = 1.f;
      }
    }
  }
}

__global__ void __launch_bounds__(256) gram_simt_kernel(const Problem* __restrict__ probs, int force) {
  const Problem& pb = probs[blockIdx.z];
  Ctrl* ctrl = pb.ctrl;
  if (!force && (ctrl->done || !ctrl->need_hess)) return;
  if (blockIdx.x > blockIdx.y) return;
  const int Dp = pb.Dp;
  const int i0 = blockIdx.y * 64, j0 = blockIdx.x * 64;
  __shared__ float Ai[16][64 + 1];
  __shared__ float Aj[16][64 + 1];
  const int tid = threadIdx.x;
  const int ti = (tid / 16) * 4, tj = (tid % 16) * 4;
  float acc[4][4] = {};
  for (long long r0 = 0; r0 < pb.n; r0 += 16) {
    for (int e = tid; e < 16 * 64; e += 256) {
      const int r = e / 64, c = e % 64;
      const long long rr = r0 + r;
      Ai[r][c] = rr < pb.n ? __bfloat162float(pb.Xt[(size_t)rr * Dp + i0 + c]) : 0.f;
      Aj[r][c] = rr < pb.n ? __bfloat162float(pb.Xt[(size_t)rr * Dp + j0 + c]) : 0.f;
    }
    __syncthreads();
#pragma unroll
    for (int r = 0; r < 16; r++) {
      float x[4], y[4];
#pragma unroll
      for (int a = 0; a < 4; a++) { x[a] = Ai[r][ti + a]; y[a] = Aj[r][tj + a]; }
#pragma unroll
      for (int a = 0; a < 4; a++)
#pragma unroll
        for (int b = 0; b < 4; b++) acc[a][b] = fmaf(x[a], y[b], acc[a][b]);
    }
    __syncthreads();
  }
  for (int s = 0; s < pb.gram_slices; s++) {
    float* out = pb.Hpart + (size_t)s * Dp * Dp;
#pragma unroll
    for (int a = 0; a < 4; a++)
#pragma unroll
      for (int b = 0; b < 4; b++) out[(size_t)(i0 + ti + a) * Dp + j0 + tj + b] = (s == 0) ? acc[a][b] : 0.f;
  }
}

typedef CUresult (*PFN_encodeTiled)(CUtensorMap*, CUtensorMapDataType, cuuint32_t, void*, const cuuint64_t*, const cuuint64_t*,
                                    const cuuint32_t*, const cuuint32_t*, CUtensorMapInterleave, CUtensorMapSwizzle,
                                    CUtensorMapL2promotion, CUtensorMapFloatOOBfill);

int gram_make_tensor_map(void* out_map_host , const void* xt, long long n, int Dp) {
  static PFN_encodeTiled fn = nullptr;
  if (!fn) {
    void* p = nullptr;
    cudaDriverEntryPointQueryResult qr;
    if (cudaGetDriverEntryPoint("cuTensorMapEncodeTiled", &p, cudaEnableDefault, &qr) != cudaSuccess || !p) return 1;
    fn = reinterpret_cast<PFN_encodeTiled>(p);
  }
  cuuint64_t dims[2] = {(cuuint64_t)Dp, (cuuint64_t)n};
  cuuint64_t strides[1] = {(cuuint64_t)Dp * 2};
  cuuint32_t box[2] = {64, (cuuint32_t)GK};
  cuuint32_t estr[2] = {1, 1};
  CUresult r = fn(reinterpret_cast<CUtensorMap*>(out_map_host), CU_TENSOR_MAP_DATA_TYPE_BFLOAT16, 2, const_cast<void*>(xt), dims,
                  strides, box, estr, CU_TENSOR_MAP_INTERLEAVE_NONE, CU_TENSOR_MAP_SWIZZLE_128B,
                  CU_TENSOR_MAP_L2_PROMOTION_L2_256B, CU_TENSOR_MAP_FLOAT_OOB_FILL_NONE);
  return r == CUDA_SUCCESS ? 0 : 2;
}

int gram_tile_list(int Dp, short* bi_bj_pairs , int max_tiles, int csr_tiles) {
  int n = 0;
  const int cols = csr_tiles ? SN : GN;
  const int nbi = (Dp + GM - 1) / GM, nbj = (Dp + cols - 1) / cols;
  for (int k = 0; k < nbi; k++) {
    const int bi = csr_tiles == 2 ? nbi - 1 - k : k;
    for (int bj = 0; bj < nbj; bj++)
      if (bj * cols <= bi * GM + GM - 1) {
        if (n >= max_tiles) return -1;
        bi_bj_pairs[2 * n] = (short)bi; bi_bj_pairs[2 * n + 1] = (short)bj; n++;
      }
  }
  return n;
}

template <typename K>
static cudaError_t set_smem_once(K kernel, size_t bytes, bool (&configured)[64]) {
  int dev = 0;
  cudaGetDevice(&dev);
  if (dev < 0 || dev >= 64 || !configured[dev]) {
    cudaError_t e = cudaFuncSetAttribute(kernel, cudaFuncAttributeMaxDynamicSharedMemorySize, (int)bytes);
    if (e != cudaSuccess) return e;
    if (dev >= 0 && dev < 64) configured[dev] = true;
  }
  return cudaSuccess;
}

cudaError_t gram_launch_wgmma(const Problem* d_probs, int nprob, const void* d_tmaps, const void* d_tiles, int ntiles,
                              int nslices, int force, cudaStream_t st, int* launches, int share) {
  static bool configured[64] = {};
  cudaError_t e = set_smem_once(gram_wgmma_kernel, G_SMEM, configured);
  if (e != cudaSuccess) return e;
  gram_wgmma_kernel<<<dim3(ntiles, nslices, nprob), G_THREADS, G_SMEM, st>>>(
      d_probs, reinterpret_cast<const CUtensorMap*>(d_tmaps), reinterpret_cast<const GramTile*>(d_tiles), ntiles, force, share);
  if (launches) *launches += 1;
  return cudaGetLastError();
}

cudaError_t gram_launch_csr_wgmma(const Problem* d_probs, int nprob, const void* d_tiles, int ntiles, int nslices, int force,
                                  cudaStream_t st, int* launches, int share) {
  static bool configured[64] = {};
  cudaError_t e = set_smem_once(gram_csr_wgmma_kernel, S_SMEM, configured);
  if (e != cudaSuccess) return e;
  gram_csr_operand_kernel<<<dim3(1024, nprob), 256, 0, st>>>(d_probs, force, share);
  if ((e = cudaGetLastError()) != cudaSuccess) return e;
  gram_csr_wgmma_kernel<<<dim3(ntiles, nslices, nprob), S_THREADS, S_SMEM, st>>>(
      d_probs, reinterpret_cast<const GramTile*>(d_tiles), ntiles, force, share);
  if (launches) *launches += 2;
  return cudaGetLastError();
}

cudaError_t gram_launch_csr_sparse(const Problem* d_probs, int nprob, const void* d_tiles, int ntiles, int force, cudaStream_t st,
                                   int* launches, int share) {
  static bool configured[64] = {};
  cudaError_t e = set_smem_once(gram_csr_sparse_kernel, SP_SMEM, configured);
  if (e != cudaSuccess) return e;
  gram_csr_operand_kernel<<<dim3(1024, nprob), 256, 0, st>>>(d_probs, force, share);
  if ((e = cudaGetLastError()) != cudaSuccess) return e;
  gram_csr_sparse_kernel<<<dim3(ntiles, 1, nprob), SP_THREADS, SP_SMEM, st>>>(d_probs, reinterpret_cast<const GramTile*>(d_tiles), force, share);
  if (launches) *launches += 2;
  return cudaGetLastError();
}

cudaError_t csr_bm_offsets(long long n, const long long* rowptr, const int* colidx, int bias_col, int nblk, long long ngroups,
                           long long* offs, cudaStream_t st) {
  const long long m = (long long)nblk * ngroups;
  cudaError_t e = cudaMemsetAsync(offs, 0, (size_t)(m + 1) * sizeof(long long), st);
  if (e != cudaSuccess) return e;
  const int grid = (int)std::min<long long>((ngroups + 7) / 8, 132 * 32);
  csr_bm_count_kernel<<<std::max(grid, 1), 256, 0, st>>>(n, rowptr, colidx, bias_col, nblk, ngroups, offs);
  if ((e = cudaGetLastError()) != cudaSuccess) return e;
  size_t tmp_bytes = 0;
  if ((e = cub::DeviceScan::ExclusiveSum(nullptr, tmp_bytes, offs, offs, (long long)(m + 1), st)) != cudaSuccess) return e;
  void* tmp = nullptr;
  if ((e = cudaMallocAsync(&tmp, tmp_bytes ? tmp_bytes : 16, st)) != cudaSuccess) return e;
  e = cub::DeviceScan::ExclusiveSum(tmp, tmp_bytes, offs, offs, (long long)(m + 1), st);
  cudaError_t e2 = cudaFreeAsync(tmp, st);
  return e != cudaSuccess ? e : e2;
}

cudaError_t csr_bm_fill(long long n, const long long* rowptr, const int* colidx, const float* vals, int bias_col, int nblk,
                        long long ngroups, const long long* offs, unsigned short* keys, float* bvals, cudaStream_t st) {
  const int grid = (int)std::min<long long>((ngroups + 7) / 8, 132 * 32);
  csr_bm_fill_kernel<<<std::max(grid, 1), 256, 0, st>>>(n, rowptr, colidx, vals, bias_col, nblk, ngroups, offs, keys, bvals);
  return cudaGetLastError();
}

cudaError_t gram_launch_simt(const Problem* d_probs, int nprob, int Dp, int force, cudaStream_t st, int* launches) {
  const int T = Dp / 64;
  gram_simt_kernel<<<dim3(T, T, nprob), 256, 0, st>>>(d_probs, force);
  if (launches) *launches += 1;
  return cudaGetLastError();
}

}
```

### ml-ease_b200/csrc/kernels.cuh

```cuda
#pragma once
#include "common.cuh"

namespace mlease {

bool k1_dense_plan(int ldx, int* R_out, int* S_out, int* G_out, size_t* smem_out, int* ctas_per_sm);
int k1_csr_window(int ldx);
cudaError_t k1_launch(const Problem* d_probs, int nprob, bool csr, int ldx, int has_bias, int ctas_per_problem,
                      int force_emit, cudaStream_t stream, int* launches, int csr_fx = 0, int nprob_dyn = 0, int mode = K1_GRAD);

bool k1f_plan(long long n, int ldx, int L, int num_sms, int* S_out, int* rows_out, int* LP_out, size_t* smem_out);
cudaError_t k1f_build(long long n, int Dg, long long nnz, const long long* rowptr, const int* colidx, const float* vals, int S, int sg_rows, int* ngrp_out,
                      int** perm_out, int** depth_out, long long** goff_out, unsigned short** row16_out, float** val_out, long long* total_out,
                      unsigned short** col16_out, cudaStream_t st);
cudaError_t k1f_launch(const Problem* d_probs, int ngroups, int L, int S, int LP, size_t smem, int has_bias, int force_emit, cudaStream_t st, int* launches,
                       int mode = K1_GRAD);
cudaError_t csr_row_l1_max(long long n, const long long* rowptr, const float* vals, unsigned* out, cudaStream_t st);

cudaError_t newton_begin(const Problem* d_probs, int nprob, double xtol, int max_newton, int hess_policy,
                         int invalidate_hess, int rebuild_is_expensive, cudaStream_t st, int* launches);
cudaError_t k1_reduce_decide(const Problem* d_probs, int nprob, int Dt, cudaStream_t st, int* launches, int spec = 0);
cudaError_t newton_solve(const Problem* d_probs, int nprob, int ldh, cudaStream_t st, int* launches, int group_L = 1);
cudaError_t newton_gemv_tri(const Problem* d_probs, int nprob, int ldh, int group_L, cudaStream_t st);
cudaError_t cg_begin(const Problem* d_probs, int nprob, cudaStream_t st, int* launches);
cudaError_t hv_reduce(const Problem* d_probs, int nprob, int Dt, int out, cudaStream_t st, int* launches);
cudaError_t cg_init(const Problem* d_probs, int nprob, int Dt, cudaStream_t st, int* launches);
cudaError_t cg_step(const Problem* d_probs, int nprob, int Dt, cudaStream_t st, int* launches);
cudaError_t cg_poll(const Problem* d_probs, int nprob, int* d_any, cudaStream_t st, int* launches);
cudaError_t newton_finish(const Problem* d_probs, int nprob, int Dt, cudaStream_t st, int* launches);

int gram_make_tensor_map(void* out_map_host, const void* xt, long long n, int Dp);
int gram_tile_list(int Dp, short* bi_bj_pairs, int max_tiles, int csr_tiles = 0);
cudaError_t gram_launch_wgmma(const Problem* d_probs, int nprob, const void* d_tmaps, const void* d_tiles, int ntiles,
                              int nslices, int force, cudaStream_t st, int* launches, int share = 0);
cudaError_t gram_launch_csr_wgmma(const Problem* d_probs, int nprob, const void* d_tiles, int ntiles, int nslices, int force,
                                  cudaStream_t st, int* launches, int share = 0);
cudaError_t gram_launch_csr_sparse(const Problem* d_probs, int nprob, const void* d_tiles, int ntiles, int force, cudaStream_t st,
                                   int* launches, int share = 0);
long long gram_sparse_max_rows();
__host__ __device__ inline int gram_sparse_span(long long entries, int nblk, long long ngroups) {
  const double per = (double)entries / ((double)(nblk > 1 ? nblk : 1) * (double)(ngroups > 1 ? ngroups : 1));
  const int g = (int)(0.75 * 448 / (per > 1.0 ? per : 1.0));
  return g < 1 ? 1 : (g > 8 ? 8 : g);
}
cudaError_t csr_bm_offsets(long long n, const long long* rowptr, const int* colidx, int bias_col, int nblk, long long ngroups, long long* offs,
                           cudaStream_t st);
cudaError_t csr_bm_fill(long long n, const long long* rowptr, const int* colidx, const float* vals, int bias_col, int nblk, long long ngroups,
                        const long long* offs, unsigned short* keys, float* bvals, cudaStream_t st);
cudaError_t gram_launch_simt(const Problem* d_probs, int nprob, int Dp, int force, cudaStream_t st, int* launches);

cudaError_t cholesky_launch(const Problem* d_probs, int nprob, int ldh, cudaStream_t st, int* launches, int share = 0, int skip_prep = 0,
                            int want_hinv = 0);
cudaError_t cholesky_prep(const Problem* d_probs, int nprob, int ldh, int share, cudaStream_t st, int* launches);
cudaError_t dmma_shapes(const double* A, const double* B, int n, int K, double* D8, double* D16, cudaStream_t st);
bool cholesky_factored_direction(int ldh);
cudaError_t cholesky_share_begin(const Problem* d_probs, int nprob, int share, cudaStream_t st, int* launches);
cudaError_t cholesky_share_end(const Problem* d_probs, int nprob, int share, cudaStream_t st, int* launches);
cudaError_t cholesky_detach_followers(const Problem* d_probs, int nprob, int ldh, cudaStream_t st, int* launches);
cudaError_t admm_reset(const Problem* d_probs, int nprob, int L, double* d_z, int ldv, const double* d_rho_eff,
                       cudaStream_t st, int* launches);
cudaError_t admm_init(const Problem* d_probs, int nprob, const double* d_z, int ldv, cudaStream_t st, int* launches);
cudaError_t admm_pack(const Problem* d_probs, int nlocal_parts, int L, int Dt, double* d_exchange, cudaStream_t st,
                      int* launches);
cudaError_t admm_consensus(const Problem* d_probs, int nlocal_parts, int L, int Dt, int ldv, int P, const double* d_exchange_sum,
                           double* d_z, const double* d_wz, const double* d_rho_eff_next, double* d_diff, cudaStream_t st,
                           int* launches, const double* d_l1_thr = nullptr);

cudaError_t postvar_rowweights(const Problem* d_probs, int nprob, const long long* d_row_start, long long nrows, int has_bias, double* d_dvec,
                               cudaStream_t st, int* launches);
cudaError_t postvar_diag(const Problem* d_probs, int nprob, const long long* d_row_start, long long nrows, const double* d_dvec, int has_bias,
                         cudaStream_t st, int* launches);
cudaError_t postvar_hessian(const Problem* d_prob, bool csr, int ldh, const double* d_dvec, const double* d_q, int has_bias, cudaStream_t st,
                            int* launches);
cudaError_t postvar_hessian_batch(const Problem* d_probs, int nprob, int ldh, const long long* d_row_start, const double* d_dvec, int has_bias,
                                  cudaStream_t st, int* launches);

}
```

Measured before the change: 52.02.

## Replace tiled sparse CSR Gram with column-indexed per-column accumulation kernel

Replaces the span/tile-based sparse CSR Gram kernel with a column-oriented kernel. At ingest, a radix sort builds a column index (offsets plus entry positions). Each CTA then takes one Gram column and accumulates that column's products into a shared-memory row of int64 sums. The operand words now pack a 20-bit column id in row-major CSR order, and the cost model that picks sparse vs WGMMA is refit with new constants. The aim is to avoid visiting empty tile/span pairs. The cost is extra ingest-time sorting and memory, plus a cap of 2^20 on column ids.

```diff
diff --git a/ml-ease_b200/csrc/batch.cu b/ml-ease_b200/csrc/batch.cu
--- a/ml-ease_b200/csrc/batch.cu
+++ b/ml-ease_b200/csrc/batch.cu
@@ -38,15 +38,14 @@
 }
 
 constexpr double GRAM_WGMMA_S_PER_MAC = 1.317e-15, GRAM_WGMMA_S_PER_READ = 4.315e-12;
-constexpr double GRAM_SPARSE_S_PER_PAIR = 1.808e-12, GRAM_SPARSE_S_PER_VISIT = 2.548e-10, GRAM_SPARSE_S_PER_READ = 2.915e-12;
-static double gram_cost(const Problem& p, int Dp, int kind, double ctas, int num_sms) {
+constexpr double GRAM_SPARSE_S_PER_PAIR = 3.084e-12, GRAM_SPARSE_S_PER_ENTRY = 1.174e-10, GRAM_SPARSE_S_PER_CELL = 5.048e-13;
+static double gram_cost(const Problem& p, int Dp, int kind, int num_sms) {
   const double nblk = Dp / 128, tiles = nblk * (nblk + 1) / 2, groups = (double)((p.n + 31) / 32);
-  const int span = gram_sparse_span(p.bm_entries, Dp / 128, (p.n + 31) / 32);
-  const double spans = (double)(((p.n + 31) / 32 + span - 1) / span);
-  const double reads = (nblk + 1) * (double)p.bm_entries;
-  if (kind == CSR_GRAM_WGMMA) return tiles * 128.0 * 128.0 * 32.0 * groups * GRAM_WGMMA_S_PER_MAC + reads * GRAM_WGMMA_S_PER_READ;
-  return (p.gram_pairs * GRAM_SPARSE_S_PER_PAIR + tiles * spans * GRAM_SPARSE_S_PER_VISIT + reads * GRAM_SPARSE_S_PER_READ) *
-         std::max(1.0, num_sms / std::max(1.0, ctas));
+  if (kind == CSR_GRAM_WGMMA)
+    return tiles * 128.0 * 128.0 * 32.0 * groups * GRAM_WGMMA_S_PER_MAC + (nblk + 1) * (double)p.bm_entries * GRAM_WGMMA_S_PER_READ;
+  const double ctas = std::min(Dp, 2 * num_sms);
+  return (p.gram_pairs * GRAM_SPARSE_S_PER_PAIR + (double)p.bm_entries * GRAM_SPARSE_S_PER_ENTRY +
+          0.5 * Dp * (Dp + 1.0) * GRAM_SPARSE_S_PER_CELL) * std::max(1.0, 2.0 * num_sms / ctas);
 }
 
 int batch_alloc(Batch& B, int num_sms, int hessian_policy, int csr_gram_force) {
@@ -92,16 +91,19 @@
   B.csr_gram = 0;
   if (B.gram_from_csr && !B.matfree) {
     double t_sparse = 0, t_wgmma = 0;
-    bool fits = true;
-    const double nblk = B.Dp / 128, ctas = nblk * (nblk + 1) / 2 * nprob;
+    bool rows_fit = true, indexed = true;
     for (auto& p : B.h) {
-      t_sparse += gram_cost(p, B.Dp, CSR_GRAM_SPARSE, ctas, num_sms);
-      t_wgmma += gram_cost(p, B.Dp, CSR_GRAM_WGMMA, ctas, num_sms);
-      if (p.n > gram_sparse_max_rows()) fits = false;
-    }
+      t_sparse += gram_cost(p, B.Dp, CSR_GRAM_SPARSE, num_sms);
+      t_wgmma += gram_cost(p, B.Dp, CSR_GRAM_WGMMA, num_sms);
+      if (p.n > gram_sparse_max_rows()) rows_fit = false;
+      if (!p.gc_pos) indexed = false;
+    }
+    const bool fits = rows_fit && indexed && B.Dt <= gram_sparse_max_cols();
     B.csr_gram = (fits && t_sparse < t_wgmma) ? CSR_GRAM_SPARSE : CSR_GRAM_WGMMA;
+    if (csr_gram_force == CSR_GRAM_SPARSE && !rows_fit)
+      return fail(MLEASE_ERR_INVALID, "the sparse CSR Gram's int64 sums hold at most 2^27 rows per partition");
     if (csr_gram_force == CSR_GRAM_SPARSE && !fits)
-      return fail(MLEASE_ERR_INVALID, "the sparse CSR Gram's int64 sums hold at most 2^27 rows per partition");
+      return fail(MLEASE_ERR_INVALID, "the sparse CSR Gram's operand word holds column ids below 2^20 (features + intercept)");
     if (csr_gram_force) B.csr_gram = csr_gram_force;
   }
   if (!B.matfree && B.csr && B.gram_from_csr) {
@@ -121,10 +123,11 @@
     B.rebuild_is_expensive = (t_rebuild > 8.0 * t_pass && B.Dt > 2048 && !B.matfree) ? 1 : 0;
   }
   constexpr int MAX_TILES = 1 << 18;
-  std::vector<short> tiles(B.matfree ? 2 : 2 * (size_t)MAX_TILES);
-  B.ntiles = B.matfree ? 0 : gram_tile_list(B.Dp, tiles.data(), MAX_TILES, B.csr_gram == CSR_GRAM_SPARSE ? 2 : B.gram_from_csr);
-  if (B.ntiles <= 0 && !B.matfree) return fail(MLEASE_ERR_INVALID, "Gram tile list overflow");
-  if (!B.matfree && B.csr_gram != CSR_GRAM_SPARSE) {
+  const bool tiled = !B.matfree && B.csr_gram != CSR_GRAM_SPARSE;
+  std::vector<short> tiles(tiled ? 2 * (size_t)MAX_TILES : 2);
+  B.ntiles = tiled ? gram_tile_list(B.Dp, tiles.data(), MAX_TILES, B.gram_from_csr) : 0;
+  if (B.ntiles <= 0 && tiled) return fail(MLEASE_ERR_INVALID, "Gram tile list overflow");
+  if (tiled) {
     const long long ksteps = (maxn + 63) / 64;
     const long long base = (long long)B.ntiles * nprob;
     const long long cap = std::max(1, num_sms);
@@ -232,7 +235,7 @@
 }
 
 cudaError_t batch_gram(const Batch& B, const Problem* d_probs, int n, int force, cudaStream_t st, int* launches, int share) {
-  if (B.csr_gram == CSR_GRAM_SPARSE) return gram_launch_csr_sparse(d_probs, n, B.d_tiles, B.ntiles, force, st, launches, share);
+  if (B.csr_gram == CSR_GRAM_SPARSE) return gram_launch_csr_sparse(d_probs, n, B.Dp, force, st, launches, share);
   if (B.gram_from_csr) return gram_launch_csr_wgmma(d_probs, n, B.d_tiles, B.ntiles, B.gram_slices, force, st, launches, share);
   return gram_launch_wgmma(d_probs, n, B.d_tmaps, B.d_tiles, B.ntiles, B.gram_slices, force, st, launches, share);
 }
diff --git a/ml-ease_b200/csrc/common.cuh b/ml-ease_b200/csrc/common.cuh
--- a/ml-ease_b200/csrc/common.cuh
+++ b/ml-ease_b200/csrc/common.cuh
@@ -72,6 +72,8 @@
   long long bm_entries;
   unsigned char* bm_e4m3;
   uint32_t* bm_word;
+  const uint32_t* gc_offs;
+  const uint32_t* gc_pos;
   float vmax, wmax;
   int nblk128;
   int sg_S, sg_rows, sg_ngrp;
diff --git a/ml-ease_b200/csrc/ingest.cu b/ml-ease_b200/csrc/ingest.cu
--- a/ml-ease_b200/csrc/ingest.cu
+++ b/ml-ease_b200/csrc/ingest.cu
@@ -207,6 +207,13 @@
     CK(csr_bm_fill(nrows, d.rowptr, d.colidx, d.vals, s->Dg, d.nblk128, d.bm_groups, bo, bk, bv, s->stream));
     d.bm_offs = bo; d.bm_keys = bk; d.bm_vals = bv;
     d.gram_pairs = (double)pairs;
+    if (nrows <= gram_sparse_max_rows() && s->Dt <= gram_sparse_max_cols()) {
+      uint32_t *co, *cp;
+      if (int rc = s->mem.get(&co, (size_t)s->Dt + 1, true)) return rc;
+      if (int rc = s->mem.get(&cp, (size_t)d.bm_entries, true)) return rc;
+      CK(csr_col_index(nrows, d.rowptr, d.colidx, s->Dg, d.bm_entries, co, cp, s->stream));
+      d.gc_offs = co; d.gc_pos = cp;
+    }
   }
   if (d.csr_unique && nnz + nrows < (1LL << 32) - 64) {
     int S = 0, rows = 0, LP = 0; size_t smem = 0;
diff --git a/ml-ease_b200/csrc/k2_gram.cu b/ml-ease_b200/csrc/k2_gram.cu
--- a/ml-ease_b200/csrc/k2_gram.cu
+++ b/ml-ease_b200/csrc/k2_gram.cu
@@ -2,6 +2,7 @@
 #include <cuda_fp8.h>
 
 #include <algorithm>
+#include <cub/device/device_radix_sort.cuh>
 #include <cub/device/device_scan.cuh>
 
 #include "kernels.cuh"
@@ -285,13 +286,10 @@
   return (b & 0x80u) ? -mag : mag;
 }
 
-constexpr uint32_t SW_VALUE_MASK = 0xFFFF8000u;
-__device__ __forceinline__ uint32_t sparse_word(uint32_t byte, int row_in_span, int col) {
-  return __float_as_uint((float)e4m3_units(byte)) | ((uint32_t)row_in_span << 7) | (uint32_t)col;
-}
-__device__ __forceinline__ int sw_units(uint32_t w) { return __float2int_rz(__uint_as_float(w & SW_VALUE_MASK)); }
-__device__ __forceinline__ int sw_row(uint32_t w) { return (int)((w >> 7) & 255u); }
-__device__ __forceinline__ int sw_col(uint32_t w) { return (int)(w & 127u); }
+constexpr uint32_t GW_VALUE_MASK = 0xFFF00000u, GW_COL_MASK = 0x000FFFFFu;
+__device__ __forceinline__ uint32_t gram_word(uint32_t byte, int col) { return __float_as_uint((float)e4m3_units(byte)) | (uint32_t)col; }
+__device__ __forceinline__ int gw_units(uint32_t w) { return __float2int_rz(__uint_as_float(w & GW_VALUE_MASK)); }
+__device__ __forceinline__ int gw_col(uint32_t w) { return (int)(w & GW_COL_MASK); }
 
 __global__ void __launch_bounds__(256) gram_csr_operand_kernel(const Problem* __restrict__ probs, int force, int share) {
   if (share > 1 && blockIdx.y % share != 0) return;
@@ -299,21 +297,36 @@
   const Ctrl* ctrl = pb.ctrl;
   if (!force && (ctrl->done || !ctrl->need_hess)) return;
   const int lane = threadIdx.x & 31;
-  const long long n = pb.n, ngroups = pb.bm_groups;
+  const long long n = pb.n;
+  const float gscale = pb.gram_scale;
+  const long long nw = ((long long)gridDim.x * blockDim.x) >> 5;
+  const long long w0 = ((long long)blockIdx.x * blockDim.x + threadIdx.x) >> 5;
+  if (pb.csr_gram == CSR_GRAM_SPARSE) {
+    const long long* __restrict__ rowptr = pb.rowptr;
+    const int* __restrict__ colidx = pb.colidx;
+    const float* __restrict__ vals = pb.vals;
+    uint32_t* __restrict__ out_w = pb.bm_word;
+    const int bias_col = pb.Dt - 1;
+    for (long long r = w0; r < n; r += nw) {
+      const float sd = pb.sdvec[r] * gscale;
+      const long long j0 = rowptr[r], j1 = rowptr[r + 1];
+      for (long long j = j0 + lane; j <= j1; j += 32) {
+        const bool bias = j == j1;
+        const uint32_t byte = __nv_cvt_float_to_fp8((bias ? 1.f : vals[j]) * sd, __NV_SATFINITE, __NV_E4M3);
+        out_w[j + r] = gram_word(byte, bias ? bias_col : colidx[j]);
+      }
+    }
+    return;
+  }
+  const long long ngroups = pb.bm_groups;
   const int nblk = pb.nblk128;
   const long long* __restrict__ offs = pb.bm_offs;
   const unsigned short* __restrict__ keys = pb.bm_keys;
   const float* __restrict__ vals = pb.bm_vals;
   unsigned char* __restrict__ out = pb.bm_e4m3;
-  uint32_t* __restrict__ out_w = pb.bm_word;
-  const bool word = pb.csr_gram == CSR_GRAM_SPARSE;
-  const int span = gram_sparse_span(pb.bm_entries, nblk, ngroups);
-  const float gscale = pb.gram_scale;
-  const long long nw = ((long long)gridDim.x * blockDim.x) >> 5;
-  for (long long g = ((long long)blockIdx.x * blockDim.x + threadIdx.x) >> 5; g < ngroups; g += nw) {
+  for (long long g = w0; g < ngroups; g += nw) {
     const long long r = g * SK + lane;
     const float sd = r < n ? pb.sdvec[r] * gscale : 0.f;
-    const int row0 = 32 * (int)(g % span);
     for (int b = 0; b < nblk; b++) {
       const uint32_t lo = (uint32_t)offs[(size_t)b * ngroups + g], hi = (uint32_t)offs[(size_t)b * ngroups + g + 1];
       for (uint32_t e0 = lo; e0 < hi; e0 += 32) {
@@ -321,186 +334,159 @@
         const bool v = e < hi;
         const uint32_t key = v ? (uint32_t)keys[e] : 0u;
         const float val = v ? vals[e] : 0.f;
-        const int k = kmaj_row(key);
-        const float sdk = __shfl_sync(0xffffffffu, sd, k);
+        const float sdk = __shfl_sync(0xffffffffu, sd, kmaj_row(key));
         const uint32_t byte = __nv_cvt_float_to_fp8(val * sdk, __NV_SATFINITE, __NV_E4M3);
-        if (!v) continue;
-        if (word) out_w[e] = sparse_word(byte, row0 + k, (int)(key >> 5));
-        else out[e] = (unsigned char)byte;
-      }
-    }
-  }
-}
-
-constexpr int SP_THREADS = 1024;
-constexpr int SP_WARPS = SP_THREADS / 32;
-constexpr int SP_SPAN = 8;
-constexpr int SP_ROWS = SP_SPAN * 32;
-constexpr int SP_AHEAD = 1;
-constexpr int SP_STAGE = 448;
-constexpr size_t SP_ACC_BYTES = (size_t)SN * SN * 2 * sizeof(uint32_t);
-constexpr size_t SP_WARP_BYTES = (size_t)SP_STAGE * 4 + (size_t)SP_ROWS * 4 + 32 * 8;
-constexpr size_t SP_SMEM = SP_ACC_BYTES + (size_t)SP_WARPS * SP_WARP_BYTES;
-static_assert(SP_SMEM <= 227 * 1024, "sparse Gram shared memory");
-static_assert(SP_STAGE % 16 == 0, "layout of the stage");
-static_assert(SP_SPAN == 8 && SP_STAGE == 448, "gram_sparse_span (kernels.cuh) assumes these");
-static_assert(SP_ROWS <= 256, "sparse_word holds the row in the span in 8 bits");
-
-__global__ void __launch_bounds__(SP_THREADS, 1)
-gram_csr_sparse_kernel(const Problem* __restrict__ probs, const GramTile* __restrict__ tiles, int force, int share) {
+        if (v) out[e] = (unsigned char)byte;
+      }
+    }
+  }
+}
+
+constexpr int GC_THREADS = 512;
+constexpr int GC_WARPS = GC_THREADS / 32;
+constexpr int GC_GROUP = 4;
+constexpr int GC_CELLS = 112 * 128;
+constexpr int GC_BIAS_UNROLL = 8;
+
+__global__ void __launch_bounds__(GC_THREADS, 2)
+gram_csr_column_kernel(const Problem* __restrict__ probs, int force, int share) {
   if (share > 1 && blockIdx.z % share != 0) return;
   const Problem& pb = probs[blockIdx.z];
   Ctrl* ctrl = pb.ctrl;
   if (!force && (ctrl->done || !ctrl->need_hess)) return;
-  const GramTile tile = tiles[blockIdx.x];
-  const int bi = tile.bi, bj = tile.bj;
-  const bool diag = bi == bj;
-  const int Dp = pb.Dp;
-  const long long ngroups = pb.bm_groups;
-  const int span = gram_sparse_span(pb.bm_entries, pb.nblk128, ngroups);
-  const long long nspans = (ngroups + span - 1) / span;
-  const int hot = diag && (pb.Dt - 1) / SN == bi ? (pb.Dt - 1) % SN : -1;
+  const int Dp = pb.Dp, Dt = pb.Dt;
+  const int hot = Dt - 1;
+  const int W = min(Dp, GC_CELLS);
+  const uint32_t nent = (uint32_t)pb.bm_entries;
+  const uint32_t* __restrict__ words = pb.bm_word;
+  const uint32_t* __restrict__ offs = pb.gc_offs;
+  const uint32_t* __restrict__ cpos = pb.gc_pos;
+  float* __restrict__ out = pb.Hpart;
 
   extern __shared__ __align__(16) unsigned char g_smem_raw[];
   uint32_t* acc_lo = reinterpret_cast<uint32_t*>(g_smem_raw);
-  int* acc_hi = reinterpret_cast<int*>(g_smem_raw) + SN * SN;
+  int* acc_hi = reinterpret_cast<int*>(g_smem_raw) + W;
   const int warp = threadIdx.x >> 5, lane = threadIdx.x & 31;
-  unsigned char* wsm = g_smem_raw + SP_ACC_BYTES + (size_t)warp * SP_WARP_BYTES;
-  int* stage = reinterpret_cast<int*>(wsm);
-  uint32_t* rtab = reinterpret_cast<uint32_t*>(wsm + SP_STAGE * 4);
-  unsigned short* rtab16 = reinterpret_cast<unsigned short*>(rtab);
-  int2* own = reinterpret_cast<int2*>(wsm + SP_STAGE * 4 + SP_ROWS * 4);
-
-  for (int e = threadIdx.x; e < SN * SN; e += SP_THREADS) { acc_lo[e] = 0u; acc_hi[e] = 0; }
+  for (int e = threadIdx.x; e < W; e += GC_THREADS) { acc_lo[e] = 0u; acc_hi[e] = 0; }
   __syncthreads();
 
-  const bool valid = bi < pb.nblk128 && bj < pb.nblk128;
-  const long long* __restrict__ offs_i = pb.bm_offs + (size_t)bi * ngroups;
-  const long long* __restrict__ offs_j = pb.bm_offs + (size_t)bj * ngroups;
-  const uint32_t* __restrict__ words = pb.bm_word;
-  const uint32_t lt = (1u << lane) - 1u;
   auto add_cell = [&](int cell, long long p) {
     const uint32_t lo = (uint32_t)p;
     const uint32_t old = atomicAdd(acc_lo + cell, lo);
     const int hi = (int)(p >> 32) + (old + lo < old ? 1 : 0);
     if (hi != 0) atomicAdd(acc_hi + cell, hi);
   };
-  auto ld_bounds = [&](long long s) -> uint32_t {
-    if (!valid || s >= nspans || lane >= 4) return 0u;
-    return (uint32_t)__ldg((lane < 2 ? offs_i : offs_j) + min(s * span + (lane & 1) * span, ngroups));
-  };
-  auto ld_entry = [&](uint32_t e, uint32_t hi) -> uint32_t { return e < hi ? __ldg(words + e) : 0u; };
-  struct Span { uint32_t ilo, ihi, jlo, jhi, i[SP_AHEAD], j[SP_AHEAD]; };
-  auto take = [&](Span& q, uint32_t b) {
-    q.ilo = __shfl_sync(0xffffffffu, b, 0); q.ihi = __shfl_sync(0xffffffffu, b, 1);
-    q.jlo = __shfl_sync(0xffffffffu, b, 2); q.jhi = __shfl_sync(0xffffffffu, b, 3);
-#pragma unroll
-    for (int k = 0; k < SP_AHEAD; k++) { q.i[k] = ld_entry(q.ilo + lane + 32 * k, q.ihi); q.j[k] = ld_entry(q.jlo + lane + 32 * k, q.jhi); }
-  };
-  long long hot_sum = 0;
-  auto run = [&](const Span& q) {
-    const uint32_t ilo = q.ilo, ihi = q.ihi, jlo = q.jlo, jhi = q.jhi;
-    if (ilo == ihi || jlo == jhi) return;
-    for (uint32_t c0 = jlo; c0 < jhi; c0 += SP_STAGE) {
-      const uint32_t c1 = min(jhi, c0 + SP_STAGE);
-      __syncwarp();
-#pragma unroll
-      for (int k = 0; k < SP_ROWS / 128; k++) reinterpret_cast<uint4*>(rtab)[lane + 32 * k] = make_uint4(0u, 0u, 0u, 0u);
-      __syncwarp();
-      int nst = 0, prev_row = -1;
-      uint32_t x[SP_AHEAD + 1];
-#pragma unroll
-      for (int k = 0; k < SP_AHEAD; k++) x[k] = c0 == jlo ? q.j[k] : ld_entry(c0 + 32 * k + lane, c1);
-      for (uint32_t base = c0; base < c1; base += 32) {
-        x[SP_AHEAD] = ld_entry(base + 32 * SP_AHEAD + lane, c1);
-        const uint32_t w = x[0];
-        const int v = sw_units(w);
-        const int r = sw_row(w);
-        const bool keep = v != 0;
-        const uint32_t m = __ballot_sync(0xffffffffu, keep);
-        const uint32_t below = m & lt;
-        const int up = __shfl_sync(0xffffffffu, r, below ? 31 - __clz(below) : 0);
-        const int pr = below ? up : prev_row;
-        const int s = nst + __popc(below);
-        if (keep) {
-          stage[s] = v * 128 + sw_col(w);
-          if (r != pr) { rtab16[2 * r] = (unsigned short)s; if (pr >= 0) rtab16[2 * pr + 1] = (unsigned short)s; }
+  auto word_at = [&](uint32_t q) -> uint32_t { return q < nent ? __ldg(words + q) : 0u; };
+
+  for (int k = blockIdx.x; k < Dp; k += gridDim.x) {
+    const int c1 = k == 0 ? hot : (k <= hot ? k - 1 : k);
+    const uint32_t p0 = c1 < Dt ? __ldg(offs + c1) : 0u, p1 = c1 < Dt ? __ldg(offs + c1 + 1) : 0u;
+    for (int w0 = c1; w0 < Dp; w0 += W) {
+      const int w1 = min(Dp, w0 + W);
+      long long hot_sum = 0;
+      if (c1 == hot) {
+        for (uint32_t i0 = p0 + threadIdx.x; i0 < p1; i0 += GC_THREADS * GC_BIAS_UNROLL) {
+          uint32_t x[GC_BIAS_UNROLL];
+#pragma unroll
+          for (int u = 0; u < GC_BIAS_UNROLL; u++) {
+            const uint32_t i = i0 + u * GC_THREADS;
+            x[u] = i < p1 ? __ldg(cpos + i) : 0xFFFFFFFFu;
+          }
+#pragma unroll
+          for (int u = 0; u < GC_BIAS_UNROLL; u++) x[u] = word_at(x[u]);
+#pragma unroll
+          for (int u = 0; u < GC_BIAS_UNROLL; u++) { const long long v = gw_units(x[u]); hot_sum += v * v; }
         }
-        if (m) prev_row = __shfl_sync(0xffffffffu, r, 31 - __clz(m));
-        nst += __popc(m);
-#pragma unroll
-        for (int k = 0; k < SP_AHEAD; k++) x[k] = x[k + 1];
-      }
-      if (nst == 0) continue;
-      if (lane == 0) rtab16[2 * prev_row + 1] = (unsigned short)nst;
-      __syncwarp();
-#pragma unroll
-      for (int k = 0; k < SP_AHEAD; k++) x[k] = q.i[k];
-      for (uint32_t base = ilo; base < ihi; base += 32) {
-        x[SP_AHEAD] = ld_entry(base + 32 * SP_AHEAD + lane, ihi);
-        const uint32_t w = x[0];
-        const int a = sw_units(w);
-        const uint32_t t = a != 0 ? rtab[sw_row(w)] : 0u;
-        const int s0 = (int)(t & 0xFFFFu), cnt = (int)(t >> 16) - s0;
-        int incl = cnt;
-#pragma unroll
-        for (int d = 1; d < 32; d <<= 1) {
-          const int u = __shfl_up_sync(0xffffffffu, incl, d);
-          if (lane >= d) incl += u;
+      } else {
+        auto walk = [&](uint32_t q, uint32_t x) {
+          const int a = gw_units(__shfl_sync(0xffffffffu, x, 0));
+          if (a == 0) return;
+          while (true) {
+            const int c2 = gw_col(x);
+            const uint32_t ends = __ballot_sync(0xffffffffu, c2 == hot);
+            uint32_t nx = 0u;
+            if (!ends) nx = word_at(q + 32 + lane);
+            const int v = gw_units(x);
+            if ((!ends || lane < __ffs(ends)) && v != 0) {
+              const long long prod = (long long)a * (long long)v;
+              if (c2 == hot) hot_sum += prod;
+              else if (c2 >= w0 && c2 < w1) add_cell(c2 - w0, prod);
+            }
+            if (ends) return;
+            x = nx;
+            q += 32;
+          }
+        };
+        for (uint32_t cb = p0 + 32u * warp; cb < p1; cb += 32u * GC_WARPS) {
+          const int cnt = (int)min(32u, p1 - cb);
+          const uint32_t mine = lane < cnt ? __ldg(cpos + cb + lane) : 0u;
+          uint32_t cur[GC_GROUP];
+#pragma unroll
+          for (int g = 0; g < GC_GROUP; g++) {
+            const uint32_t q = __shfl_sync(0xffffffffu, mine, g);
+            cur[g] = g < cnt ? word_at(q + lane) : 0u;
+          }
+          for (int j = 0; j < cnt; j += GC_GROUP) {
+            uint32_t nxt[GC_GROUP];
+#pragma unroll
+            for (int g = 0; g < GC_GROUP; g++) {
+              const int jj = j + GC_GROUP + g;
+              const uint32_t q = __shfl_sync(0xffffffffu, mine, jj & 31);
+              nxt[g] = jj < cnt ? word_at(q + lane) : 0u;
+            }
+#pragma unroll
+            for (int g = 0; g < GC_GROUP; g++) {
+              const uint32_t q = __shfl_sync(0xffffffffu, mine, j + g);
+              if (j + g < cnt) walk(q, cur[g]);
+            }
+#pragma unroll
+            for (int g = 0; g < GC_GROUP; g++) cur[g] = nxt[g];
+          }
         }
-        const int total = __shfl_sync(0xffffffffu, incl, 31);
-#pragma unroll
-        for (int k = 0; k < SP_AHEAD; k++) x[k] = x[k + 1];
-        if (total == 0) continue;
-        const uint32_t owners = __ballot_sync(0xffffffffu, cnt > 0);
-        __syncwarp();
-        if (cnt > 0) own[__popc(owners & lt)] = make_int2(a * 128 + sw_col(w), s0 - (incl - cnt));
-        __syncwarp();
-        int before = 0;
-        for (int p0 = 0; p0 < total; p0 += 32) {
-          const int end = incl - p0;
-          const uint32_t ends = __reduce_or_sync(0xffffffffu, cnt > 0 && end >= 0 && end < 32 ? 1u << end : 0u);
-          const int p = p0 + lane;
-          if (p < total) {
-            const int2 o = own[before + __popc(ends & (0xFFFFFFFFu >> (31 - lane)))];
-            const int pv = stage[p + o.y];
-            const int c1 = o.x & 127, c2 = pv & 127;
-            if (!diag || c2 <= c1) {
-              const long long prod = (long long)(o.x >> 7) * (long long)(pv >> 7);
-              if (c2 == hot && c1 == hot) hot_sum += prod;
-              else add_cell(c1 * SN + c2, prod);
-            }
-          }
-          before += __popc(ends);
-        }
-      }
-    }
-  };
-  Span cur, nxt;
-  take(cur, ld_bounds(warp));
-  uint32_t nb = ld_bounds(warp + SP_WARPS);
-  for (long long s = warp; s < nspans; s += SP_WARPS) {
-    take(nxt, nb);
-    nb = ld_bounds(s + 2 * SP_WARPS);
-    run(cur);
-    cur = nxt;
-  }
-  if (hot >= 0) {
-#pragma unroll
-    for (int d = 16; d > 0; d >>= 1) hot_sum += __shfl_down_sync(0xffffffffu, hot_sum, d);
-    if (lane == 0 && hot_sum != 0) add_cell(hot * SN + hot, hot_sum);
-  }
-  __syncthreads();
-  float* out = pb.Hpart + (size_t)bi * SN * Dp + (size_t)bj * SN;
-  for (int e = threadIdx.x; e < SN * SN; e += SP_THREADS) {
-    const int c1 = e >> 7, c2 = e & 127;
-    const int idx = diag && c2 > c1 ? c2 * SN + c1 : e;
-    const long long v = (long long)(((unsigned long long)(uint32_t)acc_hi[idx] << 32) | acc_lo[idx]);
-    out[(size_t)c1 * Dp + c2] = __ll2float_rn(v) * 0x1p-18f;
+      }
+      if (hot >= w0 && hot < w1) {
+#pragma unroll
+        for (int d = 16; d > 0; d >>= 1) hot_sum += __shfl_down_sync(0xffffffffu, hot_sum, d);
+        if (lane == 0 && hot_sum != 0) add_cell(hot - w0, hot_sum);
+      }
+      __syncthreads();
+      const int dend = (c1 / 128 + 1) * 128;
+      for (int e = threadIdx.x; e < w1 - w0; e += GC_THREADS) {
+        const int c2 = w0 + e;
+        const long long v = (long long)(((unsigned long long)(uint32_t)acc_hi[e] << 32) | acc_lo[e]);
+        acc_lo[e] = 0u; acc_hi[e] = 0;
+        const float f = __ll2float_rn(v) * 0x1p-18f;
+        out[(size_t)c2 * Dp + c1] = f;
+        if (c2 > c1 && c2 < dend) out[(size_t)c1 * Dp + c2] = f;
+      }
+      __syncthreads();
+    }
   }
 }
 
 long long gram_sparse_max_rows() { return 1LL << 27; }
+int gram_sparse_max_cols() { return 1 << 20; }
+
+__global__ void __launch_bounds__(256) csr_col_keys_kernel(long long n, const long long* __restrict__ rowptr, const int* __restrict__ colidx,
+                                                           int bias_col, uint32_t* __restrict__ keys, uint32_t* __restrict__ idx) {
+  const int lane = threadIdx.x & 31;
+  const long long nw = ((long long)gridDim.x * blockDim.x) >> 5;
+  for (long long r = ((long long)blockIdx.x * blockDim.x + threadIdx.x) >> 5; r < n; r += nw) {
+    const long long j0 = rowptr[r], j1 = rowptr[r + 1];
+    for (long long j = j0 + lane; j <= j1; j += 32) {
+      keys[j + r] = j == j1 ? (uint32_t)bias_col : (uint32_t)colidx[j];
+      idx[j + r] = (uint32_t)(j + r);
+    }
+  }
+}
+__global__ void __launch_bounds__(256) csr_col_offsets_kernel(long long entries, const uint32_t* __restrict__ sorted, int ncols,
+                                                              uint32_t* __restrict__ offs) {
+  for (long long i = (long long)blockIdx.x * blockDim.x + threadIdx.x; i <= entries; i += (long long)gridDim.x * blockDim.x) {
+    const long long lo = i == 0 ? -1 : (long long)sorted[i - 1];
+    const long long hi = i == entries ? (long long)ncols : (long long)sorted[i];
+    for (long long c = lo + 1; c <= hi; c++) offs[c] = (uint32_t)i;
+  }
+}
 
 __device__ __forceinline__ bool bias_in_block(long long r, long long n, int bias_col, int b) {
   return r < n && bias_col >= b * 128 && bias_col < b * 128 + 128;
@@ -625,8 +611,7 @@
   int n = 0;
   const int cols = csr_tiles ? SN : GN;
   const int nbi = (Dp + GM - 1) / GM, nbj = (Dp + cols - 1) / cols;
-  for (int k = 0; k < nbi; k++) {
-    const int bi = csr_tiles == 2 ? nbi - 1 - k : k;
+  for (int bi = 0; bi < nbi; bi++) {
     for (int bj = 0; bj < nbj; bj++)
       if (bj * cols <= bi * GM + GM - 1) {
         if (n >= max_tiles) return -1;
@@ -672,16 +657,52 @@
   return cudaGetLastError();
 }
 
-cudaError_t gram_launch_csr_sparse(const Problem* d_probs, int nprob, const void* d_tiles, int ntiles, int force, cudaStream_t st,
-                                   int* launches, int share) {
+cudaError_t gram_launch_csr_sparse(const Problem* d_probs, int nprob, int Dp, int force, cudaStream_t st, int* launches, int share) {
   static bool configured[64] = {};
-  cudaError_t e = set_smem_once(gram_csr_sparse_kernel, SP_SMEM, configured);
+  static int sms[64] = {};
+  cudaError_t e = set_smem_once(gram_csr_column_kernel, (size_t)GC_CELLS * 8, configured);
   if (e != cudaSuccess) return e;
+  int dev = 0, nsm = 0;
+  if ((e = cudaGetDevice(&dev)) != cudaSuccess) return e;
+  if (dev >= 0 && dev < 64 && sms[dev]) nsm = sms[dev];
+  else {
+    if ((e = cudaDeviceGetAttribute(&nsm, cudaDevAttrMultiProcessorCount, dev)) != cudaSuccess) return e;
+    if (dev >= 0 && dev < 64) sms[dev] = nsm;
+  }
   gram_csr_operand_kernel<<<dim3(1024, nprob), 256, 0, st>>>(d_probs, force, share);
   if ((e = cudaGetLastError()) != cudaSuccess) return e;
-  gram_csr_sparse_kernel<<<dim3(ntiles, 1, nprob), SP_THREADS, SP_SMEM, st>>>(d_probs, reinterpret_cast<const GramTile*>(d_tiles), force, share);
+  const size_t smem = (size_t)std::min(Dp, GC_CELLS) * 8;
+  gram_csr_column_kernel<<<dim3(std::min(Dp, 2 * nsm), 1, nprob), GC_THREADS, smem, st>>>(d_probs, force, share);
   if (launches) *launches += 2;
   return cudaGetLastError();
+}
+
+cudaError_t csr_col_index(long long n, const long long* rowptr, const int* colidx, int bias_col, long long entries, uint32_t* offs,
+                          uint32_t* pos, cudaStream_t st) {
+  cudaError_t e = cudaSuccess;
+  uint32_t *keys = nullptr, *sorted = nullptr, *idx = nullptr;
+  void* tmp = nullptr;
+  size_t tmp_bytes = 0;
+  int bits = 1;
+  while ((1LL << bits) <= bias_col) bits++;
+  auto run = [&]() -> cudaError_t {
+    cudaError_t r;
+    if ((r = cudaMallocAsync(&keys, (size_t)entries * 4, st)) != cudaSuccess) return r;
+    if ((r = cudaMallocAsync(&sorted, (size_t)entries * 4, st)) != cudaSuccess) return r;
+    if ((r = cudaMallocAsync(&idx, (size_t)entries * 4, st)) != cudaSuccess) return r;
+    const int grid = (int)std::min<long long>((n + 7) / 8, 132 * 32);
+    csr_col_keys_kernel<<<std::max(grid, 1), 256, 0, st>>>(n, rowptr, colidx, bias_col, keys, idx);
+    if ((r = cudaGetLastError()) != cudaSuccess) return r;
+    if ((r = cub::DeviceRadixSort::SortPairs(nullptr, tmp_bytes, keys, sorted, idx, pos, entries, 0, bits, st)) != cudaSuccess) return r;
+    if ((r = cudaMallocAsync(&tmp, tmp_bytes ? tmp_bytes : 16, st)) != cudaSuccess) return r;
+    if ((r = cub::DeviceRadixSort::SortPairs(tmp, tmp_bytes, keys, sorted, idx, pos, entries, 0, bits, st)) != cudaSuccess) return r;
+    csr_col_offsets_kernel<<<(int)std::min<long long>((entries + 256) / 256, 132 * 32), 256, 0, st>>>(entries, sorted, bias_col + 1, offs);
+    return cudaGetLastError();
+  };
+  e = run();
+  for (void* p : {(void*)keys, (void*)sorted, (void*)idx, tmp})
+    if (p) { cudaError_t e2 = cudaFreeAsync(p, st); if (e == cudaSuccess) e = e2; }
+  return e;
 }
 
 cudaError_t csr_bm_offsets(long long n, const long long* rowptr, const int* colidx, int bias_col, int nblk, long long ngroups,
diff --git a/ml-ease_b200/csrc/kernels.cuh b/ml-ease_b200/csrc/kernels.cuh
--- a/ml-ease_b200/csrc/kernels.cuh
+++ b/ml-ease_b200/csrc/kernels.cuh
@@ -34,14 +34,11 @@
                               int nslices, int force, cudaStream_t st, int* launches, int share = 0);
 cudaError_t gram_launch_csr_wgmma(const Problem* d_probs, int nprob, const void* d_tiles, int ntiles, int nslices, int force,
                                   cudaStream_t st, int* launches, int share = 0);
-cudaError_t gram_launch_csr_sparse(const Problem* d_probs, int nprob, const void* d_tiles, int ntiles, int force, cudaStream_t st,
-                                   int* launches, int share = 0);
+cudaError_t gram_launch_csr_sparse(const Problem* d_probs, int nprob, int Dp, int force, cudaStream_t st, int* launches, int share = 0);
 long long gram_sparse_max_rows();
-__host__ __device__ inline int gram_sparse_span(long long entries, int nblk, long long ngroups) {
-  const double per = (double)entries / ((double)(nblk > 1 ? nblk : 1) * (double)(ngroups > 1 ? ngroups : 1));
-  const int g = (int)(0.75 * 448 / (per > 1.0 ? per : 1.0));
-  return g < 1 ? 1 : (g > 8 ? 8 : g);
-}
+int gram_sparse_max_cols();
+cudaError_t csr_col_index(long long n, const long long* rowptr, const int* colidx, int bias_col, long long entries, uint32_t* offs,
+                          uint32_t* pos, cudaStream_t st);
 cudaError_t csr_bm_offsets(long long n, const long long* rowptr, const int* colidx, int bias_col, int nblk, long long ngroups, long long* offs,
                            cudaStream_t st);
 cudaError_t csr_bm_fill(long long n, const long long* rowptr, const int* colidx, const float* vals, int bias_col, int nblk, long long ngroups,
```

Result: faster. 59.29, median of 6 (+14.0%).
